# sc15i2gp/daily-ray-trace

Measured on AMD Instinct MI355X. Metric: Mpaths/s (pixels*spp/s) Cornell 1024^2 depth 8; achieved HBM GB/s % of peak, higher is better.
Workload: dtype f64

## Files before the change

daily-ray-trace_amd/csrc/drt_kernels.h:

```cpp
#pragma once

#include "drt_device.h"
#include "drt_build_rule.h"
#include "drt_stash_rule.h"
#include <type_traits>
#include "../../include/drt_hip.h"


enum
{
    SF_PX = 0, SF_PY, SF_PZ, SF_RADIUS,
    SF_NX, SF_NY, SF_NZ,
    SF_UNX, SF_UNY, SF_UNZ,
    SF_VNX, SF_VNY, SF_VNZ,
    SF_ULEN, SF_VLEN,
    SF_COUNT
};
enum
{
    LF_PX = 0, LF_PY, LF_PZ, LF_RADIUS,
    LF_UX, LF_UY, LF_UZ,
    LF_VX, LF_VY, LF_VZ,
    LF_PDF,
    LF_COUNT
// ... 1830 lines not shown
                                                     double ir, double tr, double te, double on_dot, double a_in, double spec,
                                                     double mn_dot, double ct_coef, uint32_t flags, bool paired)
{
    const uint64_t list = FIXED_N != 0u ? FIXED_LIST : list_arg;
    const uint32_t num_bdsfs = FIXED_N != 0u ? FIXED_N : num_bdsfs_arg;
    double bdsf_result = 0.0;
    double reflectance = 0.0;
#define DRT_PIN_HERE(x) asm volatile("" : "+v"(x))
    for (uint32_t i = 0; i < num_bdsfs; i += 1)
    {
        switch ((uint32_t)(list >> (4 * i)) & 15u)
        {
            case DRT_BDSF_bp_diffuse_bdsf:
                bdsf_result = diffuse_pi * a_in;
                break;
            case DRT_BDSF_bp_glossy_bdsf:
                bdsf_result = (glossy * spec) * a_in;
                break;
            case DRT_BDSF_mirror_bdsf:
                bdsf_result = (flags & FLAG_EQR) ? mirror : 0.0;
                break;
            case DRT_BDSF_fs_conductor_bdsf:
                if (SIMPLE) break;
                if (flags & FLAG_EQR)
                {
                    DRT_PIN_HERE(ir);
                    double c2 = on_dot * on_dot;
                    bdsf_result = conductor_reflectance_sel(paired, ir, tr, te, on_dot, c2, 1.0 - c2);
                }
                break;
            case DRT_BDSF_fs_dielectric_reflectance_bdsf:
                if (SIMPLE) break;
                if (flags & FLAG_EQR)
                {
                    DRT_PIN_HERE(ir);
                    bdsf_result = dielectric_reflectance_sel(paired, ir, tr, te, on_dot, 1.0 - on_dot * on_dot);
                }
                break;
            case DRT_BDSF_fs_dielectric_transmittance_bdsf:
                if (SIMPLE) break;
                if (flags & FLAG_EQT)
                {
                    DRT_PIN_HERE(ir);
                    bdsf_result = 1.0 - dielectric_reflectance_sel(paired, ir, tr, te, on_dot, 1.0 - on_dot * on_dot);
                }
                break;
            case DRT_BDSF_ct_conductor_bdsf:
            {
                if (SIMPLE) break;
                DRT_PIN_HERE(ir);
                double c2 = mn_dot * mn_dot;
                bdsf_result = conductor_reflectance_sel(paired, ir, tr, te, mn_dot, c2, 1.0 - c2) * ct_coef;
                break;
            }
            default: break;
        }
        reflectance = bdsf_result + reflectance;
    }
#undef DRT_PIN_HERE
    return reflectance;
}

#ifndef SHADE_PREFETCH_REGS
#define SHADE_PREFETCH_REGS 2
#endif
#define SHADE_PREFETCH_DEPTH 1
#define SHADE_PIXEL_CHUNK 16
#define TAIL_WINDOW_ENTRIES 112u
#define TAIL_WINDOW_WORDS (3u * TAIL_WINDOW_ENTRIES + TAIL_WINDOW_ENTRIES / 4u)
#define SHADE_WAVE_LDS_WORDS ((2u * 64u * SHADE_PREFETCH_REGS) > TAIL_WINDOW_WORDS ? (2u * 64u * SHADE_PREFETCH_REGS) : TAIL_WINDOW_WORDS)
#ifndef DRT_SHADE_CLOSED_LDS_HEADERS
#define DRT_SHADE_CLOSED_LDS_HEADERS 1
#endif
#define SHADE_CLOSED_SLOT_WORDS (64u * SHADE_PREFETCH_REGS)
#define SHADE_CLOSED_HDR01_AT SHADE_CLOSED_SLOT_WORDS
#define SHADE_CLOSED_HDR2_AT (SHADE_CLOSED_HDR01_AT + 128u)
#define SHADE_CLOSED_TAIL_ENTRIES 96u
#define SHADE_CLOSED_WAVE_LDS_WORDS (SHADE_CLOSED_HDR2_AT + 64u)
static_assert(3u * SHADE_CLOSED_TAIL_ENTRIES + SHADE_CLOSED_TAIL_ENTRIES / 4u <= SHADE_CLOSED_WAVE_LDS_WORDS, "the tail pass's window fits the closed form's region");
#define SHADE_WAVE_LDS_WORDS_FOR(closed_lds) ((closed_lds) ? SHADE_CLOSED_WAVE_LDS_WORDS : SHADE_WAVE_LDS_WORDS)

#define XYZ_FILM_WORDS 8

template <bool SPDS_IN_LDS, bool XYZ, bool SIMPLE, bool LIST = false>
__device__ __forceinline__ void shade_tail_group(const DevScene &sc, const ShadeParams &sp, const double *lds, uint64_t *wave_lds, const uint64_t *__restrict__ records,
                                                 const uint64_t *__restrict__ headers, double *__restrict__ film_pixels,
                                                 double *__restrict__ film_avgs, double *__restrict__ film_vars, uint64_t chunk_base,
                                                 uint64_t chunk_end, uint32_t lane, const bool closed, const bool closed_lds = false)
{
    const uint32_t S = sc.S;
    const uint32_t vw = sp.vertex_words;
    const uint32_t R = sp.tail_count;
    const uint32_t g = lane / R, j = lane - g * R;
    const bool act = g < (uint32_t)(chunk_end - chunk_base) && g < 64u / R;
    const uint32_t lam = sp.tail_first + j;
    const double *table = SPDS_IN_LDS ? (const double *)lds : sc.spds;
    const uint32_t n_groups = 64u / R;
    const uint32_t entries = closed_lds ? SHADE_CLOSED_TAIL_ENTRIES : TAIL_WINDOW_ENTRIES;
    const uint32_t win = entries / n_groups;
    uint16_t *task_list = (uint16_t *)(wave_lds + 3u * entries);
    const uint32_t leader = g * R;
    const bool in_group = g < n_groups;
    uint32_t v = 0, n_shaded = 0;
    uint64_t ph0 = 0;
    double vignette = 0.0, throughput = 1.0, dst = 0.0;
    uint64_t ph2 = 0;
    uint64_t slot = 0;
    const uint64_t *vcur = records;
    const bool one_light = sp.n_lights == 1u;
    const double em0 = spd_at(table, S, one_light ? sp.light0_em_spd : 0u, lam);
    auto deep_blocks = [&](uint32_t vertex) -> uint64_t { return vertex >= 2u * REC_BLOCK_VERTICES ? headers[slot * REC_HEADER_WORDS + 3] : 0ull; };
    for (uint32_t s0 = sp.tail_staged ? sp.n_samples : 0u; s0 < sp.n_samples; s0 += win)
    {
        const uint32_t s_end = s0 + win < sp.n_samples ? s0 + win : sp.n_samples;
        const uint32_t n_win = s_end - s0, n_px = (uint32_t)(chunk_end - chunk_base);
        uint32_t n_tasks = 0;
        for (uint32_t e0 = 0; e0 < n_px * n_win; e0 += 64u)
        {
            const uint32_t e = e0 + lane;
            const bool valid = e < n_px * n_win;
            const uint32_t ge = valid ? e / n_win : 0u, off = valid ? e - ge * n_win : 0u;
            const uint64_t eslot = (chunk_base + ge) * (uint64_t)sp.batch + s0 + off;
            uint64_t h0 = 0, h1 = 0, h2 = 0;
            if (valid)
            {
                const uint64_t *h = headers + eslot * REC_HEADER_WORDS;
                h0 = h[0];
                h1 = h[1];
                h2 = h[2];
            }
            const bool staged = ((uint32_t)(h0 >> 16) & HDR_TERM_TAIL_STAGED) != 0u;
            const bool has_path = valid && !staged && (h0 & 0xFFFFu) != 0u;
            if (valid && !staged && !has_path)
            {
                const bool emissive = ((uint32_t)(h0 >> 16) & HDR_TERM_MASK) == 1u;
                const uint32_t row = (uint32_t)(h0 >> 32) & 0xFFFFu;
                for (uint32_t t = 0; t < R; t += 1)
                {
                    double d = 0.0;
                    if (emissive) d = d + 1.0 * spd_at(table, S, row, sp.tail_first + t);
                    sp.tail_stage[eslot * R + t] = d * word_as_double(h1);
                }
            }
            const unsigned long long m = __ballot(has_path);
            if (has_path)
            {
                const uint32_t k = n_tasks + (uint32_t)__popcll(m & ((1ull << lane) - 1ull));
                task_list[k] = (uint16_t)e;
                uint64_t *w = wave_lds + e * 3u;
                w[0] = h0;
                w[1] = h1;
                w[2] = h2;
            }
            n_tasks += (uint32_t)__popcll(m);
        }
        __builtin_amdgcn_wave_barrier();
        uint32_t next_task = 0;
        bool busy = false;
        for (;;)
        {
            const unsigned long long want = __ballot(!busy && in_group && lane == leader);
            if (want != 0ull)
            {
                const uint32_t mine = next_task + (uint32_t)__popcll(want & ((1ull << leader) - 1ull));
                if (!busy && in_group && mine < n_tasks)
                {
                    const uint32_t e = task_list[mine];
                    const uint64_t *w = wave_lds + e * 3u;
                    const uint32_t ge = e / n_win, off = e - ge * n_win;
                    slot = (chunk_base + ge) * (uint64_t)sp.batch + s0 + off;
                    ph0 = w[0];
                    vignette = word_as_double(w[1]);
                    ph2 = w[2];
                    n_shaded = (uint32_t)(ph0 & 0xFFFFu);
                    const uint32_t k = ((uint32_t)(ph0 >> 16) >> HDR_TERM_RESUME_SHIFT) & HDR_TERM_RESUME_MASK;
                    v = k;
                    throughput = 1.0;
                    dst = 0.0;
                    if (k != 0u)
                    {
                        const double *at = sp.tail_stage + (slot * R + j);
                        dst = at[0];
                        throughput = at[shade_const().sp.tail_resume - sp.tail_stage];
                        vcur = path_vertex(records, sp.block_words, vw, ph2, deep_blocks(k), k);
                    }
                    else vcur = records + (uint64_t)(uint32_t)ph2 * sp.block_words;
                    busy = true;
                }
                next_task += (uint32_t)__popcll(want);
            }
            if (!__any(busy)) break;
            const bool has_vertex = busy && v < n_shaded;
            const bool is_plastic = has_vertex && v < 16u && (((uint32_t)(ph0 >> 48) >> v) & 1u);
            const bool is_general = has_vertex && !is_plastic;
            const uint32_t n_plastic = (uint32_t)__popcll(__ballot(is_plastic)), n_general = (uint32_t)__popcll(__ballot(is_general));
            if (n_plastic > 0 && n_plastic >= n_general)
            {
                if (is_plastic)
                {
                    const uint64_t *vrec = vcur;
                    const uint64_t w1 = vrec[1];
                    const double dir_pdf = word_as_double(vrec[4]);
                    const double s_a_in = word_as_double(vrec[5]), s_spec = word_as_double(vrec[6]);
                    const uint32_t i_diffuse = (uint32_t)(w1 >> 16) & 0xFFFFu, i_glossy = (uint32_t)(w1 >> 32) & 0xFFFFu;
                    const double diffuse_pi = spd_at(table, S, i_diffuse, lam), glossy = spd_at(table, S, i_glossy, lam);
                    double contribution = 0.0;
                    if (one_light && v < 8u)
                    {
                        if (((uint32_t)(ph0 >> 24) >> v) & 1u)
                        {
                            const uint64_t *lrec = vrec + REC_VERTEX_WORDS;
                            const double c = word_as_double(lrec[1]), a_in = word_as_double(lrec[2]), spec = word_as_double(lrec[3]);
                            double reflectance = diffuse_pi * a_in + 0.0;
                            reflectance = (glossy * spec) * a_in + reflectance;
                            contribution = contribution + reflectance;
                            contribution = contribution * em0;
                            contribution = contribution * c;
                        }
                    }
                    else if (one_light)
                    {
                        const uint64_t *lrec = vrec + REC_VERTEX_WORDS;
                        const uint64_t lw0 = lrec[0];
                        const double c = word_as_double(lrec[1]), a_in = word_as_double(lrec[2]), spec = word_as_double(lrec[3]);
                        double reflectance = diffuse_pi * a_in + 0.0;
                        reflectance = (glossy * spec) * a_in + reflectance;
                        double lit = 0.0 + reflectance;
                        lit = lit * em0;
                        lit = lit * c;
                        contribution = ((uint32_t)(lw0 >> 16) & FLAG_VISIBLE) ? lit : 0.0;
                    }
                    else
                    for (uint32_t l = 0; l < sp.n_lights; l += 1)
                    {
                        const uint64_t *lrec = vrec + REC_VERTEX_WORDS + l * REC_LIGHT_WORDS;
                        const uint64_t lw0 = lrec[0];
                        if (!((uint32_t)(lw0 >> 16) & FLAG_VISIBLE)) continue;
                        const double c = word_as_double(lrec[1]), a_in = word_as_double(lrec[2]), spec = word_as_double(lrec[3]);
                        double reflectance = diffuse_pi * a_in + 0.0;
                        reflectance = (glossy * spec) * a_in + reflectance;
                        contribution = contribution + reflectance;
                        contribution = contribution * spd_at(table, S, (uint32_t)(lw0 & 0xFFFFu), lam);
                        contribution = contribution * c;
                    }
                    dst = dst + throughput * contribution;
                    double reflectance = diffuse_pi * s_a_in + 0.0;
                    reflectance = (glossy * s_spec) * s_a_in + reflectance;
                    reflectance = reflectance * dir_pdf;
                    throughput = throughput * reflectance;
                    v += 1;
                    if (v < n_shaded) vcur = (v & (REC_BLOCK_VERTICES - 1u)) != 0u ? vcur + vw : path_vertex(records, sp.block_words, vw, ph2, deep_blocks(v), v);
                }
            }
            else if (n_general > 0)
            {
                if (is_general)
                {
                    const uint64_t *vrec = vcur;
                    const uint64_t list = vrec[0], w1 = vrec[1], w2 = vrec[2];
                    const double on_dot = word_as_double(vrec[3]), dir_pdf = word_as_double(vrec[4]);
                    const uint32_t num_bdsfs = (uint32_t)(w1 & 0xFFu);
                    const uint32_t sflags = (uint32_t)(w1 >> 8) & 0xFFu;
                    const uint32_t i_diffuse = (uint32_t)(w1 >> 16) & 0xFFFFu, i_glossy = (uint32_t)(w1 >> 32) & 0xFFFFu;
                    const double diffuse_pi = spd_at(table, S, i_diffuse, lam), glossy = spd_at(table, S, i_glossy, lam);
                    const double mirror = spd_at(table, S, (uint32_t)(w1 >> 48) & 0xFFFFu, lam);
                    uint32_t f0, f1, f2;
                    bool paired;
                    fresnel_rows(w2, f0, f1, f2, paired);
                    const double ir = SIMPLE ? 0.0 : spd_at(table, S, f0, lam), tr = SIMPLE ? 0.0 : spd_at(table, S, f1, lam), te = SIMPLE ? 0.0 : spd_at(table, S, f2, lam);
                    auto lane_vertex = [&](auto eval) {
                        double contribution = 0.0;
                        for (uint32_t l = 0; l < sp.n_lights; l += 1)
                        {
                            const uint64_t *lrec = vrec + REC_VERTEX_WORDS + l * REC_LIGHT_WORDS;
                            const uint64_t lw0 = lrec[0];
                            const uint32_t lflags = (uint32_t)(lw0 >> 16) & 0xFFu;
                            if (!(lflags & FLAG_VISIBLE)) continue;
                            double reflectance = eval(lflags, lrec + 2);
                            contribution = contribution + reflectance;
                            contribution = contribution * spd_at(table, S, (uint32_t)(lw0 & 0xFFFFu), lam);
                            contribution = contribution * word_as_double(lrec[1]);
                        }
                        dst = dst + throughput * contribution;
                        double reflectance = eval(sflags, vrec + 5);
                        reflectance = reflectance * dir_pdf;
                        throughput = throughput * reflectance;
                    };
                    const bool glass = !SIMPLE && num_bdsfs == 2u && list == DRT_LIST_GLASS;
                    const bool ggx = closed && list == DRT_LIST_GGX;
                    if (glass)
                        lane_vertex([&](uint32_t flags, const uint64_t *) {
                            return bdsf_at_wavelength<SIMPLE, 2, DRT_LIST_GLASS>(0, 0, 0.0, 0.0, 0.0, ir, tr, te, on_dot, 0.0, 0.0, 0.0, 0.0, flags, paired);
                        });
                    else if (ggx)
                        lane_vertex([&](uint32_t flags, const uint64_t *a) {
                            return bdsf_at_wavelength<SIMPLE, 1, DRT_LIST_GGX>(0, 0, 0.0, 0.0, 0.0, ir, tr, te, 0.0, 0.0, 0.0, word_as_double(a[2]), word_as_double(a[3]), flags, paired);
                        });
                    else if (closed && list == DRT_LIST_MIRROR)
                        lane_vertex([&](uint32_t flags, const uint64_t *) {
                            return bdsf_at_wavelength<SIMPLE, 1, DRT_LIST_MIRROR>(0, 0, 0.0, 0.0, mirror, 0.0, 0.0, 0.0, 0.0, 0.0, 0.0, 0.0, 0.0, flags, false);
                        });
                    else if (closed && list == DRT_LIST_CONDUCTOR)
                        lane_vertex([&](uint32_t flags, const uint64_t *) {
                            return bdsf_at_wavelength<SIMPLE, 1, DRT_LIST_CONDUCTOR>(0, 0, 0.0, 0.0, 0.0, ir, tr, te, on_dot, 0.0, 0.0, 0.0, 0.0, flags, paired);
                        });
                    else if (closed)
                        lane_vertex([&](uint32_t flags, const uint64_t *a) {
                            return bdsf_at_wavelength<SIMPLE, 2, DRT_LIST_PLASTIC>(0, 0, diffuse_pi, glossy, 0.0, 0.0, 0.0, 0.0, 0.0, word_as_double(a[0]), word_as_double(a[1]), 0.0, 0.0, flags, false);
                        });
                    else
                        lane_vertex([&](uint32_t flags, const uint64_t *a) {
                            return bdsf_at_wavelength<SIMPLE>(list, num_bdsfs, diffuse_pi, glossy, mirror, ir, tr, te, on_dot, word_as_double(a[0]), word_as_double(a[1]),
                                                              word_as_double(a[2]), word_as_double(a[3]), flags, paired);
                        });
                    v += 1;
                    if (v < n_shaded) vcur = (v & (REC_BLOCK_VERTICES - 1u)) != 0u ? vcur + vw : path_vertex(records, sp.block_words, vw, ph2, deep_blocks(v), v);
                }
            }
            if (busy && v >= n_shaded)
            {
                if (((uint32_t)(ph0 >> 16) & HDR_TERM_MASK) == 1u) dst = dst + throughput * spd_at(table, S, (uint32_t)(ph0 >> 32) & 0xFFFFu, lam);
                sp.tail_stage[slot * R + j] = dst * vignette;
                busy = false;
            }
        }
        __builtin_amdgcn_wave_barrier();
    }
    uint32_t j_b = j;
    asm volatile("" : "+v"(j_b));
    const uint32_t lam_b = sp.tail_first + j_b;
    uint32_t g_b = g;
    asm volatile("" : "+v"(g_b));
    const uint64_t pix_b = chunk_base + g_b;
    const uint64_t pix_f = LIST ? (act ? (uint64_t)sp.pixel_list[pix_b] : 0u) : pix_b;
    double *px = film_pixels + pix_f * (uint64_t)(XYZ ? XYZ_FILM_WORDS : S + 1);
    double *pa = XYZ ? nullptr : film_avgs + pix_f * (uint64_t)S;
    double *pv = XYZ ? nullptr : film_vars + pix_f * (uint64_t)S;
    const double *stage = sp.tail_stage + (pix_b * (uint64_t)sp.batch) * R + j_b;
    const uint32_t first = LIST ? sp.first_sample + (act ? sp.sample_base[pix_f] : 0u) : sp.first_sample;
    double f_sum = (act && !XYZ) ? px[lam_b] : 0.0, f_avg = (act && !XYZ) ? pa[lam_b] : 0.0, f_var = (act && !XYZ) ? pv[lam_b] : 0.0;
#pragma unroll 4
    for (uint32_t k = 0; k < sp.n_samples; k += 1)
    {
        const double contribution = act ? stage[(uint64_t)k * R] : 0.0;
        const double denom = (double)(first + k + 1);
        f_sum = f_sum + contribution;
        if (!XYZ)
        {
            double t0 = contribution - f_avg;
            double t1 = t0;
            t0 = t0 / denom;
            f_avg = f_avg + t0;
            t0 = contribution - f_avg;
            t0 = t1 * t0;
            f_var = f_var + t0;
        }
    }
    if (XYZ)
    {
        const double rw = spd_at(table, S, sp.cmf_rw, lam_b);
        const double x = act ? (spd_at(table, S, sp.cmf_x, lam_b) * f_sum * rw) : 0.0;
        const double y = act ? (spd_at(table, S, sp.cmf_y, lam_b) * f_sum * rw) : 0.0;
        const double z = act ? (spd_at(table, S, sp.cmf_z, lam_b) * f_sum * rw) : 0.0;
        double X = 0.0, Y = 0.0, Z = 0.0;
        for (uint32_t t = 0; t < R; t += 1)
        {
            const int src = (int)((lane - j_b + t) & 63u);
            X += __shfl(x, src);
            Y += __shfl(y, src);
            Z += __shfl(z, src);
        }
        if (act && j_b == 0)
        {
            px[4] += X;
            px[5] += Y;
            px[6] += Z;
        }
    }
    else if (act)
    {
        px[lam_b] = f_sum;
        pa[lam_b] = f_avg;
        pv[lam_b] = f_var;
    }
}


template <int NSETS, bool SPDS_IN_LDS, bool XYZ, bool DARK, bool SIMPLE, bool LIST, bool CLOSED, bool CLOSED_LDS = false>
__device__ __forceinline__ void shade_pixels(const DevScene &sc, const ShadeParams &sp, const uint64_t *__restrict__ records,
                                             const uint64_t *__restrict__ headers, double *__restrict__ film_pixels,
                                             double *__restrict__ film_avgs, double *__restrict__ film_vars,
                                             unsigned long long *__restrict__ work_counter)
{
    static_assert(!CLOSED || (NSETS == 1 && SPDS_IN_LDS && !XYZ && !SIMPLE && !LIST), "the closed form exists for one wavelength set, tables in LDS, spectral film, dense launches");
    extern __shared__ double lds[];
    const uint32_t S = sc.S;
    if (*sp.overflow) return;
    if (SPDS_IN_LDS)
    {
        const uint32_t spd_words = sc.n_spd * S;
        for (uint32_t k = threadIdx.x; k < spd_words; k += SHADE_BLOCK) lds[k] = sc.spds[k];
        __syncthreads();
    }
    const uint32_t lane_k = threadIdx.x & 63u;
    static_assert(!CLOSED_LDS || CLOSED, "the form with headers in LDS is a closed form");
    constexpr bool LDS_HDR = CLOSED_LDS;
    uint64_t *rec_lds = (uint64_t *)(lds + (SPDS_IN_LDS ? (size_t)sc.n_spd * S : 0)) + (size_t)(threadIdx.x >> 6) * SHADE_WAVE_LDS_WORDS_FOR(LDS_HDR);
    const uint32_t vw = sp.vertex_words;
    const uint32_t vpr = vw <= 64 ? 64u / vw : 0u;
    const uint32_t n_fast_regs = vpr * SHADE_PREFETCH_REGS;
    const uint32_t n_fast = n_fast_regs < 2u * REC_BLOCK_VERTICES ? n_fast_regs : 2u * REC_BLOCK_VERTICES;

    uint32_t lam_c[NSETS];
#pragma unroll
    for (int k = 0; k < NSETS; k += 1)
    {
        const uint32_t lam = 64u * k + lane_k;
        lam_c[k] = lam < S ? lam : 0;
    }

    const uint32_t S_main = sp.tail_count ? sp.tail_first : S;
    for (;;)
    {
        const ShadeParams &qc = shade_const().sp;
        uint32_t item = 0;
        if (lane_k == 0) item = (uint32_t)atomicAdd(work_counter, 1ull);
        item = (uint32_t)__builtin_amdgcn_readfirstlane((int)item);
        if (item >= qc.n_items) break;
        const uint32_t lane = made_again<LDS_HDR>(lane_k);
        if constexpr (LDS_HDR) lam_c[0] = lane < S ? lane : 0;
        const bool split = qc.items_per_group > 1;
        const bool inline_tail = qc.tail_count != 0;
        const uint32_t mains_per_group = qc.items_per_group - (inline_tail ? 1u : 0u);
        bool tail_item = inline_tail;
        uint32_t group = item, sub = 0;
        if (split)
        {
            uint32_t m = item;
            if (inline_tail)
            {
                const uint32_t n_groups = qc.n_items / qc.items_per_group;
                const uint32_t q = qc.tail_period_mains, mixed = n_groups * (q + 1u);
                if (item < mixed)
                {
                    const uint32_t period = item / (q + 1u), r = item - period * (q + 1u);
                    tail_item = r == 0u;
                    group = period;
                    m = period * q + (r - 1u);
                }
                else
                {
                    tail_item = false;
                    m = n_groups * q + (item - mixed);
                }
            }
            if (!tail_item)
            {
                group = m / mains_per_group;
                sub = m - group * mains_per_group;
            }
        }
        const uint64_t chunk_base = (uint64_t)group * qc.chunk;
        const uint64_t chunk_end = (chunk_base + qc.chunk < qc.n_pix) ? chunk_base + qc.chunk : qc.n_pix;
        uint64_t main_base = chunk_base, main_end = chunk_end;
        if (split)
        {
            main_base = chunk_base + (uint64_t)sub * qc.sub_pixels;
            main_end = (main_base + qc.sub_pixels < chunk_end) ? main_base + qc.sub_pixels : chunk_end;
            if (tail_item || main_base > chunk_end) main_base = main_end = chunk_end;
        }

      if (qc.mode == 2u) main_base = main_end;
      for (uint64_t pix = main_base; pix < main_end; pix += 1)
      {

        const uint64_t pix_f = LIST ? (uint64_t)sp.pixel_list[pix] : pix;
        double *px = film_pixels + pix_f * (uint64_t)(XYZ ? XYZ_FILM_WORDS : S + 1);
        double *pa = XYZ ? nullptr : film_avgs + pix_f * (uint64_t)S;
        double *pv = XYZ ? nullptr : film_vars + pix_f * (uint64_t)S;
        const uint32_t first = LIST ? sp.first_sample + sp.sample_base[pix_f] : sp.first_sample;
        double f_sum[NSETS], f_avg[NSETS], f_var[NSETS];
#pragma unroll
        for (int k = 0; k < NSETS; k += 1)
        {
            const uint32_t lam = 64u * k + lane;
            const bool active = lam < S_main;
            f_sum[k] = (active && !XYZ) ? px[lam] : 0.0;
            f_avg[k] = (active && !XYZ) ? pa[lam] : 0.0;
            f_var[k] = (active && !XYZ) ? pv[lam] : 0.0;
        }
        bool dark = false;
        if (DARK)
        {
            bool some = false;
#pragma unroll
            for (int k = 0; k < NSETS; k += 1)
                some = some || ((uint64_t)__double_as_longlong(f_sum[k]) | (uint64_t)__double_as_longlong(f_avg[k]) | (uint64_t)__double_as_longlong(f_var[k])) != 0ull;
            dark = !__any(some);
        }
      for (uint32_t s0 = 0; s0 < sp.n_samples; s0 += 64u)
      {
        const uint32_t n_win = (uint32_t)__builtin_amdgcn_readfirstlane((int)((sp.n_samples - s0 < 64u) ? sp.n_samples - s0 : 64u));
        __builtin_assume(n_win >= 1u);
        uint64_t h0 = 0, h1 = 0, h2 = 0, h3 = 0;
        if (lane < n_win)
        {
            const uint64_t *h = headers + (pix * sp.batch + s0 + lane) * REC_HEADER_WORDS;
            h0 = h[0];
            h1 = h[1];
            h2 = h[2];
            if (!LDS_HDR) h3 = h[3];
        }
        const unsigned long long worthless = !DARK ? 0ull : __ballot(lane < n_win && (h0 & 0xFFFFu) == 0ull && ((uint32_t)(h0 >> 16) & HDR_TERM_MASK) != 1u &&
                                                                      __builtin_isfinite(word_as_double(h1)));
        if (DARK && dark && (uint32_t)__popcll(worthless) == n_win) continue;
        auto prefetch_blocks = [&](uint64_t b2, uint32_t nw, uint64_t *dst) __attribute__((always_inline)) {
#pragma unroll
            for (int k = 0; k < SHADE_PREFETCH_REGS; k += 1)
            {
                const uint32_t b = (64u * k) >> (sp.vertex_shift + REC_BLOCK_SHIFT);
                const uint32_t id = b == 0 ? (uint32_t)b2 : (uint32_t)(b2 >> 32);
                const uint64_t *base = records + (uint64_t)id * sp.block_words + (64u * k - (b << (sp.vertex_shift + REC_BLOCK_SHIFT)));
                dst[k] = (64u * k + lane < nw) ? base[lane] : 0;
            }
        };
        auto prefetch = [&](uint32_t sa, uint32_t nw, uint64_t *dst) {
            if (nw == 0u) return;
            prefetch_blocks(readlane64(h2, sa), nw, dst);
        };
        uint64_t ring[SHADE_PREFETCH_DEPTH + 1][SHADE_PREFETCH_REGS];
        const uint64_t *hdr01 = rec_lds + SHADE_CLOSED_HDR01_AT, *hdr2 = rec_lds + SHADE_CLOSED_HDR2_AT;
        uint64_t hs_v = 0, vig_v = 0, nx0_v = 0, nx2_v = 0;
        auto fetch_headers = [&](uint32_t t) {
            const uint32_t a = t & 63u, b = (t + 1u) & 63u;
            hs_v = hdr01[a];
            vig_v = hdr01[64u + a];
            nx0_v = hdr01[b];
            nx2_v = hdr2[b];
        };
        if constexpr (LDS_HDR)
        {
            static_assert(SHADE_PREFETCH_DEPTH == 1, "one sample ahead");
            __builtin_amdgcn_wave_barrier();
            uint64_t *hw = rec_lds + SHADE_CLOSED_HDR01_AT;
            hw[lane] = h0;
            hw[64u + lane] = h1;
            hw[128u + lane] = h2;
            __builtin_amdgcn_wave_barrier();
            fetch_headers(0u);
            const uint64_t head0 = first64(hs_v);
            const uint32_t nw = (uint32_t)(head0 & 0xFFFFu) * vw;
            if (nw != 0u) prefetch_blocks(first64(hdr2[0]), nw, ring[1]);
        }
        else
        {
#pragma unroll
        for (int d = 0; d < SHADE_PREFETCH_DEPTH; d += 1)
        {
            const uint32_t nw = ((uint32_t)d < n_win) ? (uint32_t)(readlane64(h0, d) & 0xFFFFu) * vw : 0u;
            prefetch((uint32_t)d < n_win ? (uint32_t)d : 0u, nw, ring[d + 1]);
        }
        }
        for (uint32_t s = 0; s < n_win; s += 1)
        {
            const uint64_t hs = LDS_HDR ? first64(hs_v) : readlane64(h0, s);
            const uint64_t vig_w = LDS_HDR ? vig_v : readlane64(h1, s);
            const double vignette = word_as_double(vig_w);
            const uint32_t n_shaded = (uint32_t)(hs & 0xFFFFu);
            const uint32_t term = (uint32_t)(hs >> 16) & HDR_TERM_MASK;
// ... 399 lines not shown
                    for (int k = 0; k < NSETS; k += 1)
                    {
                        double reflectance = bdsf_at_wavelength<SIMPLE>(list, num_bdsfs, diffuse[k], glossy[k], mirror[k], ir[k], tr[k], te[k], on_dot,
                                                                word_as_double(lw[2]), word_as_double(lw[3]), word_as_double(lw[4]),
                                                                word_as_double(lw[5]), lflags, paired);
                        contribution[k] = contribution[k] + reflectance;
                        contribution[k] = contribution[k] * spd_at(table, S, i_em, lam_c[k]);
                        contribution[k] = contribution[k] * c;
                    }
                }
                const double s_mn = lifted_double<LDS_HDR>(vslot + 7, src, lane0 + 7), s_ct = lifted_double<LDS_HDR>(vslot + 8, src, lane0 + 8);
#pragma unroll
                for (int k = 0; k < NSETS; k += 1)
                {
                    dst[k] = dst[k] + throughput[k] * contribution[k];
                    double reflectance = bdsf_at_wavelength<SIMPLE>(list, num_bdsfs, diffuse[k], glossy[k], mirror[k], ir[k], tr[k], te[k], on_dot,
                                                            s_a_in, s_spec, s_mn, s_ct, sflags, paired);
                    reflectance = reflectance * dir_pdf;
                    throughput[k] = throughput[k] * reflectance;
                }
            }
            if constexpr (LDS_HDR) fetch_headers(s + 1u);
            const double denom = (double)(first + s0 + s + 1);
            if (DARK) dark = false;
#pragma unroll
            for (int k = 0; k < NSETS; k += 1)
            {
                if (term == 1)
                {
                    const double em = SPDS_IN_LDS ? spd_at((const double *)lds, S, term_spd, lam_c[k]) : spd_at(sc.spds, S, term_spd, lam_c[k]);
                    dst[k] = dst[k] + throughput[k] * em;
                }
                const double contribution = dst[k] * vignette;
                f_sum[k] = f_sum[k] + contribution;
                if (!XYZ)
                {
                    double t0 = contribution - f_avg[k];
                    double t1 = t0;
                    t0 = t0 / denom;
                    f_avg[k] = f_avg[k] + t0;
                    t0 = contribution - f_avg[k];
                    t0 = t1 * t0;
                    f_var[k] = f_var[k] + t0;
                }
            }
        }
      }
        if (XYZ)
        {
            const double *table = SPDS_IN_LDS ? (const double *)lds : sc.spds;
            double X = 0.0, Y = 0.0, Z = 0.0;
#pragma unroll
            for (int k = 0; k < NSETS; k += 1)
            {
                const uint32_t lam = 64u * k + lane;
                if (lam < S_main)
                {
                    const double rw = spd_at(table, S, sp.cmf_rw, lam);
                    X += (spd_at(table, S, sp.cmf_x, lam) * f_sum[k] * rw);
                    Y += (spd_at(table, S, sp.cmf_y, lam) * f_sum[k] * rw);
                    Z += (spd_at(table, S, sp.cmf_z, lam) * f_sum[k] * rw);
                }
            }
            for (int off = 32; off > 0; off >>= 1)
            {
                X += __shfl_xor(X, off);
                Y += __shfl_xor(Y, off);
                Z += __shfl_xor(Z, off);
            }
            if (lane == 0)
            {
                px[0] += X;
                px[1] += Y;
                px[2] += Z;
                px[3] += (double)sp.n_samples * 1.0;
            }
        }
        else
        {
#pragma unroll
            for (int k = 0; k < NSETS; k += 1)
            {
                const uint32_t lam = 64u * k + lane;
                if (lam < S_main)
                {
                    px[lam] = f_sum[k];
                    pa[lam] = f_avg[k];
                    pv[lam] = f_var[k];
                }
            }
            if (lane == 0) px[S] += (double)sp.n_samples * 1.0;
        }
      }

        if constexpr (LDS_HDR)
        {
            __builtin_amdgcn_wave_barrier();
        }
        if (tail_item && sp.mode != 1u) shade_tail_group<SPDS_IN_LDS, XYZ, SIMPLE, LIST>(sc, sp, (const double *)lds, rec_lds, records, headers, film_pixels, film_avgs, film_vars, chunk_base, chunk_end, made_again<LDS_HDR>(lane), CLOSED, LDS_HDR);
    }
}

template <int NSETS, bool SPDS_IN_LDS, bool XYZ, bool DARK, bool SIMPLE = false, bool LIST = false>
__global__ __launch_bounds__(SHADE_BLOCK, (SIMPLE && NSETS == 1) ? DRT_SHADE_WAVES_SIMPLE : SHADE_WAVES_PER_SIMD_FOR(NSETS)) void drt_shade_kernel(DevScene sc, ShadeParams sp, const uint64_t *__restrict__ records,
                                                                 const uint64_t *__restrict__ headers, double *__restrict__ film_pixels,
                                                                 double *__restrict__ film_avgs, double *__restrict__ film_vars,
                                                                 unsigned long long *__restrict__ work_counter)
{
    shade_pixels<NSETS, SPDS_IN_LDS, XYZ, DARK, SIMPLE, LIST, false>(sc, sp, records, headers, film_pixels, film_avgs, film_vars, work_counter);
}

#ifndef DRT_SHADE_WAVES_CLOSED
#define DRT_SHADE_WAVES_CLOSED 4
#endif
template <bool DARK>
__global__ __launch_bounds__(SHADE_BLOCK, DRT_SHADE_WAVES_CLOSED) void drt_shade_kernel_closed(DevScene sc, ShadeParams sp, const uint64_t *__restrict__ records,
                                                                 const uint64_t *__restrict__ headers, double *__restrict__ film_pixels,
                                                                 double *__restrict__ film_avgs, double *__restrict__ film_vars,
                                                                 unsigned long long *__restrict__ work_counter)
{
    shade_pixels<1, true, false, DARK, false, false, true>(sc, sp, records, headers, film_pixels, film_avgs, film_vars, work_counter);
}

#ifndef DRT_SHADE_WAVES_CLOSED_LDS
#define DRT_SHADE_WAVES_CLOSED_LDS 5
#endif
#if DRT_SHADE_CLOSED_LDS_HEADERS
template <bool DARK>
__global__ __launch_bounds__(SHADE_BLOCK, DRT_SHADE_WAVES_CLOSED_LDS) void drt_shade_kernel_closed_lds(DevScene sc, ShadeParams sp, const uint64_t *__restrict__ records,
                                                                 const uint64_t *__restrict__ headers, double *__restrict__ film_pixels,
                                                                 double *__restrict__ film_avgs, double *__restrict__ film_vars,
                                                                 unsigned long long *__restrict__ work_counter)
{
    shade_pixels<1, true, false, DARK, false, false, true, true>(sc, sp, records, headers, film_pixels, film_avgs, film_vars, work_counter);
}
#endif

__global__ void drt_film_xyz_kernel(DevScene sc, uint32_t cmf_rw, uint32_t cmf_x, uint32_t cmf_y, uint32_t cmf_z, double interval,
                                    uint64_t n_pix, const double *__restrict__ film_pixels, double *__restrict__ xyz)
{
    uint64_t p = (uint64_t)blockIdx.x * blockDim.x + threadIdx.x;
    if (p >= n_pix) return;
    const uint32_t S = sc.S;
    const double *rw = sc.spds + (size_t)cmf_rw * S, *cx = sc.spds + (size_t)cmf_x * S;
    const double *cy = sc.spds + (size_t)cmf_y * S, *cz = sc.spds + (size_t)cmf_z * S;
    const double *px = film_pixels + p * (uint64_t)(S + 1);
    double f = px[S];
    double n = 0.0;
    for (uint32_t i = 0; i < S; i += 1) n += (cy[i] * rw[i]);
    n *= interval;
    double X = 0.0, Y = 0.0, Z = 0.0;
    for (uint32_t i = 0; i < S; i += 1)
    {
        double v = px[i] / f;
        X += (cx[i] * v * rw[i]);
        Y += (cy[i] * v * rw[i]);
        Z += (cz[i] * v * rw[i]);
    }
    xyz[3 * p + 0] = X * (interval / n);
    xyz[3 * p + 1] = Y * (interval / n);
    xyz[3 * p + 2] = Z * (interval / n);
}

__global__ void drt_film_bgra_kernel(DevScene sc, uint32_t cmf_rw, uint32_t cmf_x, uint32_t cmf_y, uint32_t cmf_z, double interval,
                                     uint64_t n_pix, const double *__restrict__ film, int which, uint8_t *__restrict__ bgra)
{
    uint64_t p = (uint64_t)blockIdx.x * blockDim.x + threadIdx.x;
    if (p >= n_pix) return;
    const uint32_t S = sc.S;
    const double *rw = sc.spds + (size_t)cmf_rw * S, *cx = sc.spds + (size_t)cmf_x * S;
    const double *cy = sc.spds + (size_t)cmf_y * S, *cz = sc.spds + (size_t)cmf_z * S;
    const double *px = film + p * (uint64_t)(which == 0 ? S + 1 : S);
    double div = 1.0;
    bool divide = false;
    if (which == 0) { div = px[S]; divide = true; }
    if (which == 2)
    {
        double highest = 0.0;
        for (uint32_t i = 0; i < S; i += 1) if (px[i] > highest) highest = px[i];
        div = highest;
        divide = true;
    }
    double n = 0.0;
    for (uint32_t i = 0; i < S; i += 1) n += (cy[i] * rw[i]);
    n *= interval;
    double X = 0.0, Y = 0.0, Z = 0.0;
    for (uint32_t i = 0; i < S; i += 1)
    {
        double v = divide ? px[i] / div : px[i];
        X += (cx[i] * v * rw[i]);
        Y += (cy[i] * v * rw[i]);
        Z += (cz[i] * v * rw[i]);
    }
    X *= (interval / n);
    Y *= (interval / n);
    Z *= (interval / n);
    double rgb[3];
    rgb[0] = (2.3706743 * X) - (0.9000405 * Y) - (0.4706338 * Z);
    rgb[1] = (-0.5138850 * X) + (1.4253036 * Y) + (0.0885814 * Z);
    rgb[2] = (0.0052982 * X) - (0.0146949 * Y) + (1.0093968 * Z);
    uint8_t out[3];
    for (int c = 0; c < 3; c += 1)
    {
        double f = rgb[c];
        f = (f < 0.0) ? 0.0 : f;
        f = (f > 1.0) ? 1.0 : f;
        out[c] = (f == f) ? (uint8_t)(f * 255.0) : (uint8_t)0;
    }
    uchar4 o;
    o.x = out[2]; o.y = out[1]; o.z = out[0]; o.w = 255;
    ((uchar4 *)bgra)[p] = o;
}

__global__ void drt_xyz_finish_kernel(DevScene sc, uint32_t cmf_rw, uint32_t cmf_y, double interval, uint64_t n_pix,
                                      const double *__restrict__ film, double *__restrict__ xyz)
{
    uint64_t p = (uint64_t)blockIdx.x * blockDim.x + threadIdx.x;
// ... 313 lines not shown
```

daily-ray-trace_amd/csrc/drt_launcher.hip:

```cpp
#include "drt_kernels.h"
#include "drt_bvh_kernels.h"
#include "drt_adaptive_kernels.h"
#include "drt_sample_map_kernels.h"
#include "drt_denoise_kernels.h"
#include "drt_feature_kernels.h"
#include "drt_matte_kernels.h"
#include "drt_ray_kernels.h"
#include "drt_update_kernels.h"
#include "drt_build_kernels.h"
#include "drt_material_kernels.h"
#include "drt_depth_kernels.h"
#include "drt_sensor_kernels.h"
#include "drt_bucket_kernels.h"
#include "drt_lobe_kernels.h"
#include "drt_window_kernels.h"
#include "drt_window_rule.h"
#include "drt_pair_rule.h"
#include "drt_shade_lds_rule.h"
#include "drt_owned.h"

#include <algorithm>
#include <cmath>
#include <cstdarg>
#include <cstdio>
// ... 32 lines not shown

struct DeviceMem
{
    static std::atomic<uint64_t> &live() { static std::atomic<uint64_t> n{0}; return n; }
    static hipError_t alloc(void **p, size_t bytes)
    {
        const hipError_t e = hipMalloc(p, bytes);
        if (e == hipSuccess) live() += 1;
        return e;
    }
    static void free(void *p) { (void)hipFree(p); live() -= 1; }
};
struct PinnedMem
{
    static std::atomic<uint64_t> &live() { static std::atomic<uint64_t> n{0}; return n; }
    static hipError_t alloc(void **p, size_t bytes)
    {
        const hipError_t e = hipHostMalloc(p, bytes, hipHostMallocDefault);
        if (e == hipSuccess) live() += 1;
        return e;
    }
    static void free(void *p) { (void)hipHostFree(p); live() -= 1; }
};
template <typename T> using DevBuf = Owned<T, DeviceMem>;
template <typename T> using PinnedBuf = Owned<T, PinnedMem>;

struct drt_context
{
    int         device = 0;
    hipStream_t stream = nullptr;
    Stream      own_stream;
    drt_params  params{};
    DevScene    dsc{};
    DevCamera   dcam{};
    uint32_t    cmf_rw = 0, cmf_x = 0, cmf_y = 0, cmf_z = 0;
    double      interval = 0.0;

    std::vector<DevBuf<unsigned char>> allocations;
    std::vector<DevMaterial> host_mats;
    DevMaterial *d_mat_variants = nullptr;
    double *d_pixels = nullptr, *d_avgs = nullptr, *d_vars = nullptr;
    DevBuf<double> own_pixels, own_avgs, own_vars;
    bool    xyz_mode = false;
    bool    own_film = false;
    DevBuf<uint64_t> d_records, d_headers;
    uint32_t  light0_em_spd = 0;
    DevBuf<double> d_tail_stage;
    DevBuf<double> d_tail_resume;
    uint32_t  batch_spp = 1;
    uint32_t  vertex_words = 0, vertex_shift = 0, block_words = 0;
    uint64_t  pool_blocks = 0;
    uint32_t  worst_blocks_per_path = 0;
    double    est_blocks_per_path = 0.0;
    struct Batch { PairSpan span; uint64_t seq; };
    std::vector<Batch> inflight;
    uint64_t  next_seq = 1;
    uint64_t  redone_batches = 0, pool_peak = 0;
    DevBuf<int32_t> d_hits;
    uint64_t  hits_capacity = 0;
    uint32_t  hits_samples = 0;
    DevBuf<unsigned long long> d_counters;
    DevBuf<PrimaryHit> d_primary;
    DevBuf<uint64_t> d_queue;
    bool        bvh_pipeline = false;
    int         primary_grid_cap = 0, bounce_grid_cap = 0;
    DevBuf<double> d_xyz;
    DevBuf<uint8_t> d_bgra;
    bool      trace_tail = false;
    bool      tail_all_staged = false;
    bool      tail_resume = false;
    bool      dark_skip = true;
    bool      dark_skip_win = true;
    bool      no_fixed_lists = false;
    bool      simple_bdsfs = false;
    bool      no_closed_shade = false;
    bool      closed_lists = false;
    const double *d_spd_tail = nullptr;

    bool   scene_in_lds = true, spds_in_lds = true, use_bvh = false;
    size_t trace_lds = 0, shade_lds = 0;
    size_t shade_lds_closed = 0;
    bool   closed_lds = false;
    bool trace_stash = false;
    int    trace_grid_cap = 0, shade_grid_cap = 0;
    uint32_t trace_chunk_override = 0;
    ShadeOverrides shade_overrides;
    uint32_t debug_shade_mode = 0;
    bool     debug_tail_phase_a_off = false;
    uint32_t shade_sets = 1, tail_first = 0, tail_count = 0;
    uint64_t n_pix = 0;

    std::vector<Event> ev;
    std::vector<double> ev_paths;
    size_t ev_used = 0;
    double trace_ms = 0.0, shade_ms = 0.0;
    uint64_t timed_pairs = 0;
    double min_sample_ms = 0.0, max_sample_ms = 0.0, avg_sample_ms = 0.0;

    bool film_used = false, adaptive_done = false;
    DevBuf<uint32_t> d_counts;
    DevBuf<uint32_t> d_alist[2];
    DevBuf<unsigned long long> d_keep;
    DevBuf<uint32_t> d_bkeep;
    DevBuf<uint32_t> d_ainfo;
    PinnedBuf<uint32_t> h_active;
    uint64_t film_gen = 0;
    uint64_t dn_gen = 0;
    bool     dn_valid = false;
    DevBuf<double> d_dn_mean, d_dn_var, d_dn_guide, d_dn_weights, d_dn_wsum;
    DevBuf<uint32_t> d_dn_unusable;
    uint32_t dn_window_cap = 0;
    std::vector<drt_material> ft_mats;
    std::vector<double> ft_spds;
    uint32_t ft_n_spd = 0, ft_S = 0;
    DevBuf<double> d_ft_mean, d_ft_m2, d_ft_colour;
    DevBuf<int32_t> d_ft_ids;
    DevBuf<uint32_t> d_ft_counts, d_ft_report;
    DevBuf<unsigned long long> d_ft_info;
    Event    ft_ev[2];
    bool     ft_valid = false, ft_from_film = false;
    uint64_t ft_gen = 0;
    DevBuf<int32_t> d_mt_ids, d_mt_list;
    DevBuf<uint32_t> d_mt_counts, d_mt_tail;
    DevBuf<double> d_mt_cover;
    DevBuf<unsigned long long> d_mt_info;
    Event    mt_ev[2];
    bool     mt_valid = false, mt_from_film = false;
    uint64_t mt_gen = 0;
    uint64_t ray_chunk = RAY_STAGING_RAYS;
    int      ray_grid_cap = 1;
    DevBuf<double> d_ray_a, d_ray_b;
    DevBuf<drt_ray_hit> d_ray_hits;
    DevBuf<uint8_t> d_ray_visible;
    DevBuf<uint32_t> d_ray_xy, d_ray_samples;
    bool        rays_bound = false;
    DevRayTable rt{};
    DevBuf<double> d_rt_origins, d_rt_dirs, d_rt_weights;
    std::vector<drt_surface> h_surfaces;
    bool      h_stale = false;
    std::vector<BvhNode>  h_nodes;
    std::vector<uint32_t> h_order;
    double    cam_reach = 0.0, extent = 0.0;
    bool      extent_known = true;
    bool      upd_ready = false;
    DevBuf<drt_surface> d_raw; PinnedBuf<drt_surface> h_stage;
    DevBuf<int32_t> d_light_slot;
    DevBuf<double> d_boxes;
    DevBuf<uint32_t> d_leaf_parent;
    DevBuf<uint2> d_levels;
    std::vector<uint32_t> level_first;
    DevBuf<unsigned long long> d_upd_status;
    Event     upd_ev[3];
    bool      upd_timed = false, stage_busy = false;
    bool      upd_check = false, upd_violation = false;
    uint32_t  updates = 0, refits = 0;
    double    upd_ms = 0.0;
    bool      boxes_valid = false;
    bool      hb_ready = false, hb_timed = false;
    bool      hb_mirror_pending = false;
    DevBuf<uint32_t> d_hb_tree_surf, d_hb_pos[2], d_hb_table, d_hb_order;
    DevBuf<uint64_t> d_hb_keys[2];
    DevBuf<uint4> d_hb_items[2];
    DevBuf<unsigned char> d_hb_status; PinnedBuf<unsigned char> hb_mirror;
    Event     hb_ev[3];
    uint32_t  hb_builds = 0, hb_built_by = 0, hb_depth = 0;
    double    hb_ms = 0.0;
// ... 518 lines not shown
    if (ctx->use_bvh)
    {
        BvhBuilder bb;
        bb.build(scene, reach);
        if (bb.max_depth > BVH_STACK) return fail(-2, "BVH of %zu surfaces is %d levels deep, the traversal stack holds %d", bb.prims.size(), bb.max_depth, BVH_STACK);
        if (!(bb.extent < 134217728.0)) return fail(-2, "scene or camera coordinates reach %g: the hierarchy's f32 box test holds up to 2^27", bb.extent);
        std::vector<BvhLeafPrim> leaf(std::max<size_t>(bb.order.size(), 1));
        memset(leaf.data(), 0, leaf.size() * sizeof(BvhLeafPrim));
        for (size_t k = 0; k < bb.order.size(); k += 1)
        {
            const uint32_t i = bb.order[k];
            leaf[k].index = i;
            leaf[k].type = stype[i];
            for (int f = 0; f < 4; f += 1) leaf[k].f[f] = surf[(size_t)f * n_surf + i];
            leaf[k].reach32 = INFINITY;
            if (stype[i] == DRT_GEO_SPHERE)
            {
                for (int f = 0; f < 3; f += 1) leaf[k].c32[f] = (float)leaf[k].f[f];
                leaf[k].reach32 = bvh_sphere_reach32(leaf[k].f[3], bb.extent);
            }
        }
        if ((rc = upload(ctx, bb.nodes, &d.bvh_nodes))) return rc;
        if ((rc = upload(ctx, leaf, &d.bvh_leaf))) return rc;
        ctx->h_nodes = bb.nodes;
        ctx->h_order = bb.order;
        ctx->hb_depth = (uint32_t)bb.max_depth;
        ctx->extent = bb.extent;
    }
    if (!ctx->scene_in_lds) ctx->trace_lds = 0;
    ctx->spds_in_lds = (size_t)d.n_spd * S * 8 <= 64 * 1024;
    {
        uint32_t sets = 0, tf = 0, tc = 0;
        shade_sets(S, &sets, &tf, &tc);
        const size_t extra = (size_t)d.n_spd * tc * 8 + (size_t)(TRACE_BLOCK / 64) * (2 * tc + 1) * 64 * 8;
        ctx->simple_bdsfs = !getenv("DRT_NO_SIMPLE_SHADE");
        ctx->no_fixed_lists = getenv("DRT_NO_FIXED_LISTS") != nullptr;
        for (uint32_t i = 0; i < scene->num_materials; i += 1)
            for (uint32_t j = 0; j < mats[i].num_bdsfs; j += 1)
            {
                const uint32_t b = mats[i].bdsfs[j];
                if (b != DRT_BDSF_bp_diffuse_bdsf && b != DRT_BDSF_bp_glossy_bdsf && b != DRT_BDSF_mirror_bdsf) ctx->simple_bdsfs = false;
            }
        ctx->no_closed_shade = getenv("DRT_NO_CLOSED_SHADE") != nullptr;
        ctx->closed_lists = closed_lists(mats.data(), scene->num_materials, smat.data(), n_surf);
        bool all_simple = true;
        for (uint32_t i = 0; i < n_surf; i += 1)
        {
            const DevMaterial &m = mats[smat[i]];
            const bool mirror_only = m.num_bdsfs == 1u && m.bdsfs[0] == DRT_BDSF_mirror_bdsf;
            if (!(m.is_black_body || (m.vertex_flags & FLAG_PLASTIC) || mirror_only)) all_simple = false;
        }
        const char *e = getenv("DRT_TRACE_TAIL");
        const size_t lane_rows = (size_t)(TRACE_BLOCK / 64) * (TRACE_LANE_ROWS + 1) * 64 * 8;
        ctx->trace_tail = ctx->scene_in_lds && sets == 1 && tc > 0 && tc <= 8 && n_lights == 1 && ctx->trace_lds + extra - lane_rows <= 48 * 1024 && !(e && *e == '0') &&
                          (all_simple || !(e && *e == '2'));
        ctx->tail_all_staged = ctx->trace_tail && all_simple;
        const char *er = getenv("DRT_TAIL_RESUME");
        ctx->tail_resume = ctx->trace_tail && !ctx->tail_all_staged && !(er && *er == '0');
        if (ctx->trace_tail)
        {
            std::vector<double> cols((size_t)d.n_spd * tc);
            for (uint32_t r = 0; r < d.n_spd; r += 1)
                for (uint32_t j = 0; j < tc; j += 1) cols[(size_t)r * tc + j] = spds[(size_t)r * S + tf + j];
            if ((rc = upload(ctx, cols, &ctx->d_spd_tail))) return rc;
            ctx->trace_lds += extra;
        }
    }
    return 0;
}

static bool shade_simple(const drt_context *ctx) { return ctx->simple_bdsfs && ctx->spds_in_lds && ctx->shade_sets == 1; }

static bool shade_dark(const drt_context *ctx, const ShadeParams &sp)
{
    return (ctx->win_open && !sp.pixel_list) ? ctx->dark_skip_win : ctx->dark_skip;
}

static bool shade_closed(const drt_context *ctx)
{
    return ctx->closed_lists && !ctx->no_closed_shade && !ctx->no_fixed_lists && !shade_simple(ctx) && ctx->spds_in_lds && ctx->shade_sets == 1 && !ctx->xyz_mode;
}

static bool shade_closed_lds(const drt_context *ctx) { return DRT_SHADE_CLOSED_LDS_HEADERS != 0 && ctx->closed_lds && shade_closed(ctx); }

template <int NSETS, bool XYZ, bool LIST>
static int launch_shade_mode(drt_context *ctx, uint32_t grid, const ShadeParams &sp, double *const film[3])
{
    if (NSETS == 1 && !XYZ && !LIST && shade_closed(ctx))
    {
#define DRT_LAUNCH_CLOSED(KERNEL, DARK, LDS_BYTES)                                                                                                 \
    hipLaunchKernelGGL((KERNEL<DARK>), dim3(grid), dim3(SHADE_BLOCK), LDS_BYTES, ctx->stream, ctx->dsc, sp, ctx->d_records, \
                       ctx->d_headers, film[0], film[1], film[2], ctx->d_counters + DRT_NUM_COUNTERS + 1)
#if DRT_SHADE_CLOSED_LDS_HEADERS
        if (shade_closed_lds(ctx))
        {
            if (shade_dark(ctx, sp)) DRT_LAUNCH_CLOSED(drt_shade_kernel_closed_lds, true, ctx->shade_lds_closed);
            else DRT_LAUNCH_CLOSED(drt_shade_kernel_closed_lds, false, ctx->shade_lds_closed);
            return 0;
        }
#endif
        if (shade_dark(ctx, sp)) DRT_LAUNCH_CLOSED(drt_shade_kernel_closed, true, ctx->shade_lds);
        else DRT_LAUNCH_CLOSED(drt_shade_kernel_closed, false, ctx->shade_lds);
#undef DRT_LAUNCH_CLOSED
        return 0;
    }
#define DRT_LAUNCH_SHADE(LDS, DARK, SIMPLE)                                                                                                       \
    hipLaunchKernelGGL((drt_shade_kernel<NSETS, LDS, XYZ, DARK, SIMPLE, LIST>), dim3(grid), dim3(SHADE_BLOCK), ctx->shade_lds, ctx->stream, ctx->dsc, sp, \
                       ctx->d_records, ctx->d_headers, film[0], film[1], film[2], ctx->d_counters + DRT_NUM_COUNTERS + 1)
    if (NSETS == 1 && shade_simple(ctx))
    {
        if (shade_dark(ctx, sp)) DRT_LAUNCH_SHADE(true, true, (NSETS == 1));
        else DRT_LAUNCH_SHADE(true, false, (NSETS == 1));
    }
    else if (ctx->spds_in_lds && shade_dark(ctx, sp)) DRT_LAUNCH_SHADE(true, true, false);
    else if (ctx->spds_in_lds) DRT_LAUNCH_SHADE(true, false, false);
    else if (shade_dark(ctx, sp)) DRT_LAUNCH_SHADE(false, true, false);
    else DRT_LAUNCH_SHADE(false, false, false);
#undef DRT_LAUNCH_SHADE
    return 0;
}

template <int NSETS>
static int launch_shade_sets(drt_context *ctx, uint32_t grid, const ShadeParams &sp, double *const film[3])
{
    if (sp.pixel_list) return launch_shade_mode<NSETS, false, true>(ctx, grid, sp, film);
    return ctx->xyz_mode ? launch_shade_mode<NSETS, true, false>(ctx, grid, sp, film) : launch_shade_mode<NSETS, false, false>(ctx, grid, sp, film);
}

static void shade_sets(uint32_t S, uint32_t *n_sets, uint32_t *tail_first, uint32_t *tail_count)
{
    uint32_t full = S / 64, rem = S % 64;
    *tail_first = 0;
    *tail_count = 0;
    if (S <= 64 || rem == 0) *n_sets = (S + 63) / 64;
    else if (rem <= 16 && !getenv("DRT_NO_TAIL_PASS"))
    {
        *n_sets = full;
        *tail_first = 64 * full;
        *tail_count = rem;
    }
    else *n_sets = full + 1;
}

static int launch_shade(drt_context *ctx, uint32_t grid, const ShadeParams &sp, double *const film[3])
{
    switch (ctx->shade_sets)
    {
        case 1: return launch_shade_sets<1>(ctx, grid, sp, film);
        case 2: return launch_shade_sets<2>(ctx, grid, sp, film);
        case 3: return launch_shade_sets<3>(ctx, grid, sp, film);
        default: return launch_shade_sets<4>(ctx, grid, sp, film);
    }
}

template <int NCUTS>
static const void *depth_kernel(bool lds) { return lds ? (const void *)drt_depth_cut_kernel<NCUTS, true> : (const void *)drt_depth_cut_kernel<NCUTS, false>; }
static const void *depth_kernel(uint32_t n_cuts, bool lds)
{
    switch (n_cuts)
    {
        case 1: return depth_kernel<1>(lds);
        case 2: return depth_kernel<2>(lds);
        case 3: return depth_kernel<3>(lds);
        case 4: return depth_kernel<4>(lds);
        case 5: return depth_kernel<5>(lds);
        case 6: return depth_kernel<6>(lds);
        case 7: return depth_kernel<7>(lds);
        default: return depth_kernel<8>(lds);
    }
}
static size_t depth_lds_bytes(const drt_context *ctx) { return ctx->spds_in_lds ? (size_t)ctx->dsc.n_spd * ctx->dsc.S * 8 : 0; }

static int launch_depth_cuts(drt_context *ctx, const ShadeParams &sp, uint64_t pix0)
{
    const size_t S = ctx->dsc.S;
    DepthCutParams dp{};
// ... 321 lines not shown
    ctx->ft_spds.assign(scene->spds, scene->spds + (size_t)scene->num_spds * scene->num_wavelengths);
    if (const char *e = getenv("DRT_NO_LIVE_WINDOW")) ctx->win_allowed = atoi(e) == 0;
    if (ctx->xyz_mode)
    {
        const uint32_t rows[4] = {scene->cmf_rw, scene->cmf_x, scene->cmf_y, scene->cmf_z};
        for (int k = 0; k < 4; k += 1)
            for (uint32_t i = 0; i < scene->num_wavelengths; i += 1)
                if (!std::isfinite(scene->spds[(size_t)rows[k] * scene->num_wavelengths + i])) ctx->win_allowed = false;
    }

    set_device_camera(ctx, camera);

    const uint32_t S = scene->num_wavelengths;
    ctx->n_pix = (uint64_t)params->tile_w * params->tile_h;
    ctx->vertex_words = 16;
    while (ctx->vertex_words < REC_VERTEX_WORDS + REC_LIGHT_WORDS * ctx->dsc.n_lights) ctx->vertex_words *= 2;
    ctx->vertex_shift = 0;
    while ((1u << ctx->vertex_shift) < ctx->vertex_words) ctx->vertex_shift += 1;
    ctx->block_words = REC_BLOCK_VERTICES * ctx->vertex_words;
    const uint32_t deepest = (params->max_depth + REC_BLOCK_VERTICES - 1) / REC_BLOCK_VERTICES;
    ctx->worst_blocks_per_path = deepest + (deepest > REC_HEADER_BLOCKS ? 1u : 0u);
    if (deepest > REC_HEADER_BLOCKS + 2 * ctx->block_words)
        return fail(-2, "max_depth %u: a path's table block holds %u blocks beyond the header's %d", params->max_depth, 2 * ctx->block_words, REC_HEADER_BLOCKS);
    if (ctx->dsc.n_spd >= 0xFFFFu) return fail(-2, "too many SPDs for the 16-bit record indices");
    if (S > 64 * SHADE_MAX_SETS) return fail(-2, "more than %d wavelengths", 64 * SHADE_MAX_SETS);
    {
        uint32_t sets = 0, tf = 0, tc = 0;
        shade_sets(S, &sets, &tf, &tc);
        ctx->tail_count = tc;
    }
    ctx->bvh_pipeline = !ctx->scene_in_lds;

    HIP_TRY(ctx->own_pixels.need(pixels_bytes(ctx) / 8));
    if (!ctx->xyz_mode)
    {
        HIP_TRY(ctx->own_avgs.need((size_t)ctx->n_pix * S));
        HIP_TRY(ctx->own_vars.need((size_t)ctx->n_pix * S));
    }
    ctx->d_pixels = ctx->own_pixels;
    ctx->d_avgs = ctx->own_avgs;
    ctx->d_vars = ctx->own_vars;
    ctx->own_film = true;
    HIP_TRY(hipMemsetAsync(ctx->d_pixels, 0, pixels_bytes(ctx), ctx->stream));
    if (ctx->d_avgs) HIP_TRY(hipMemsetAsync(ctx->d_avgs, 0, (size_t)ctx->n_pix * S * 8, ctx->stream));
    if (ctx->d_vars) HIP_TRY(hipMemsetAsync(ctx->d_vars, 0, (size_t)ctx->n_pix * S * 8, ctx->stream));
    HIP_TRY(ctx->d_counters.need(DRT_COUNTER_WORDS));
    HIP_TRY(hipMemsetAsync(ctx->d_counters, 0, DRT_COUNTER_WORDS * sizeof(unsigned long long), ctx->stream));

    hipDeviceProp_t prop;
    HIP_TRY(hipGetDeviceProperties(&prop, ctx->device));
    int per_cu = 0;
    if (ctx->scene_in_lds && ctx->trace_tail)
        HIP_TRY(hipOccupancyMaxActiveBlocksPerMultiprocessor(&per_cu, drt_trace_direct_kernel<true, true>, TRACE_BLOCK, ctx->trace_lds));
    else if (ctx->scene_in_lds)
        HIP_TRY(hipOccupancyMaxActiveBlocksPerMultiprocessor(&per_cu, drt_trace_direct_kernel<true, false>, TRACE_BLOCK, ctx->trace_lds));
    ctx->trace_stash = false;
    if (ctx->scene_in_lds && !(getenv("DRT_NO_RAY_STASH") && atoi(getenv("DRT_NO_RAY_STASH")) != 0) && ctx->trace_lds + TRACE_STASH_BYTES <= 64 * 1024)
    {
        int with = 0;
        if (ctx->trace_tail) HIP_TRY(hipOccupancyMaxActiveBlocksPerMultiprocessor(&with, drt_trace_kernel<true, true>, TRACE_BLOCK, ctx->trace_lds + TRACE_STASH_BYTES));
        else HIP_TRY(hipOccupancyMaxActiveBlocksPerMultiprocessor(&with, drt_trace_kernel<true, false>, TRACE_BLOCK, ctx->trace_lds + TRACE_STASH_BYTES));
        ctx->trace_stash = with >= 1 && with >= per_cu;
    }
    if (per_cu < 1) per_cu = 1;
    if (const char *e = getenv("DRT_TRACE_BLOCKS_PER_CU")) per_cu = std::max(1, atoi(e));
    ctx->trace_grid_cap = prop.multiProcessorCount * per_cu;
    ctx->ray_grid_cap = prop.multiProcessorCount * 4;
    if (const char *e = getenv("DRT_RAY_CHUNK"))
        ctx->ray_chunk = std::max<uint64_t>(1, std::min<uint64_t>(RAY_STAGING_RAYS, strtoull(e, nullptr, 0)));
    if (ctx->bvh_pipeline)
    {
        int p_cu = 0, b_cu = 0;
        HIP_TRY(hipOccupancyMaxActiveBlocksPerMultiprocessor(&p_cu, drt_primary_kernel<false>, PRIMARY_BLOCK, 0));
        HIP_TRY(hipOccupancyMaxActiveBlocksPerMultiprocessor(&b_cu, drt_bounce_kernel<false>, BOUNCE_BLOCK, 0));
        if (const char *e = getenv("DRT_TRACE_BLOCKS_PER_CU")) b_cu = std::max(1, atoi(e));
        ctx->primary_grid_cap = prop.multiProcessorCount * std::max(1, p_cu);
        ctx->bounce_grid_cap = prop.multiProcessorCount * std::max(1, b_cu);
    }
    const ShadeLdsPlan lds_general = shade_lds_plan(ctx->dsc.n_spd, S, ctx->spds_in_lds, SHADE_WAVES, SHADE_WAVE_LDS_WORDS_FOR(false), DRT_SHADE_WAVES_PER_SIMD);
    const ShadeLdsPlan lds_closed = shade_lds_plan(ctx->dsc.n_spd, S, ctx->spds_in_lds, SHADE_WAVES, SHADE_WAVE_LDS_WORDS_FOR(true), DRT_SHADE_WAVES_CLOSED_LDS);
    ctx->shade_lds = lds_general.group_bytes;
    ctx->shade_lds_closed = lds_closed.group_bytes;
    ctx->closed_lds = lds_closed.groups >= DRT_SHADE_WAVES_CLOSED_LDS * SHADE_SIMDS_PER_CU / SHADE_WAVES && getenv("DRT_NO_CLOSED_LDS") == nullptr;
    int s_per_cu = 0;
    shade_sets(S, &ctx->shade_sets, &ctx->tail_first, &ctx->tail_count);
    switch (ctx->shade_sets)
    {
        case 1: rc = shade_occupancy<1>(ctx, &s_per_cu); break;
        case 2: rc = shade_occupancy<2>(ctx, &s_per_cu); break;
        case 3: rc = shade_occupancy<3>(ctx, &s_per_cu); break;
        default: rc = shade_occupancy<4>(ctx, &s_per_cu); break;
    }
    if (rc) return rc;
    const int s_query = s_per_cu;
    if (shade_closed_lds(ctx)) s_per_cu = std::min(s_per_cu, (int)lds_closed.groups);
    if (s_per_cu < 1) s_per_cu = 1;
    if (const char *e = getenv("DRT_SHADE_BLOCKS_PER_CU")) s_per_cu = std::max(1, atoi(e));
    ctx->shade_grid_cap = prop.multiProcessorCount * s_per_cu;
    if (const char *e = getenv("DRT_RESERVE_BLOCKS"))
    {
        int n = std::max(0, atoi(e));
        ctx->trace_grid_cap = std::max(1, ctx->trace_grid_cap - n);
        ctx->shade_grid_cap = std::max(1, ctx->shade_grid_cap - n);
    }
    if (const char *e = getenv("DRT_TRACE_CHUNK")) ctx->trace_chunk_override = (uint32_t)std::min(1 << 20, std::max(64, atoi(e) / 64 * 64));
    if (const char *e = getenv("DRT_TAIL_PERIOD")) ctx->shade_overrides.tail_period = (uint32_t)std::max(0, atoi(e));
    if (const char *e = getenv("DRT_SHADE_SUBS")) ctx->shade_overrides.subs = (uint32_t)std::max(0, atoi(e));
    if (const char *e = getenv("DRT_SHADE_CHUNK")) ctx->shade_overrides.chunk = (uint32_t)atoi(e);
    if (const char *e = getenv("DRT_DEBUG_SHADE_MODE")) ctx->debug_shade_mode = (uint32_t)atoi(e);
    if (const char *e = getenv("DRT_DEBUG_TAIL_PHASE_A_OFF")) ctx->debug_tail_phase_a_off = atoi(e) != 0;
    const size_t block_bytes = (size_t)ctx->block_words * 8;
    const uint64_t npx = std::max<uint64_t>(ctx->n_pix, 1);
    const size_t per_path_fixed = REC_HEADER_WORDS * 8 + (size_t)ctx->tail_count * 8 * (ctx->tail_resume ? 2 : 1) +
                                  (ctx->bvh_pipeline ? sizeof(PrimaryHit) + sizeof(uint64_t) : 0);
    size_t free_b = 0, total_b = 0;
    HIP_TRY(hipMemGetInfo(&free_b, &total_b));
    ctx->est_blocks_per_path = (double)ctx->worst_blocks_per_path;
    if (npx * (uint64_t)ctx->worst_blocks_per_path * block_bytes > (256ull << 20) && !getenv("DRT_POOL_WORST_CASE"))
    {
        const bool win = window_in_use(ctx);
        const PairWindow pw = {win, ctx->wx0, ctx->wx1, ctx->wy0, ctx->wy1};
        const uint64_t live_px = win ? (uint64_t)(ctx->wx1 - ctx->wx0) * (ctx->wy1 - ctx->wy0) : npx;
        const TraceTile sample = pool_sample_tile(ctx->params, pw, pool_sample_step(live_px));
        const uint64_t n_sample = sample.n_pix;
        ctx->pool_blocks = blocks_worst_case(ctx, n_sample);
        HIP_TRY(ctx->d_records.need(ctx->pool_blocks * ctx->block_words));
        HIP_TRY(ctx->d_headers.need(n_sample * REC_HEADER_WORDS));
        if (ctx->bvh_pipeline)
        {
            HIP_TRY(ctx->d_primary.need(n_sample));
            HIP_TRY(ctx->d_queue.need(n_sample));
        }
        if ((rc = enqueue_trace(ctx, sample, PairSpan::whole_tile(ctx->params.first_sample, 1, 0)))) return rc;
        unsigned long long used = 0;
        HIP_TRY(hipMemcpyAsync(&used, ctx->d_counters + DRT_PAIR_COUNTERS + 5, sizeof(used), hipMemcpyDeviceToHost, ctx->stream));
        HIP_TRY(hipStreamSynchronize(ctx->stream));
        ctx->est_blocks_per_path = (double)used / (double)n_sample * ((double)live_px / (double)npx);
        {
            unsigned long long cnt[3] = {0, 0, 0};
            HIP_TRY(hipMemcpy(cnt, ctx->d_counters + DRT_PAIR_COUNTERS, sizeof(cnt), hipMemcpyDeviceToHost));
            if (cnt[0] > 0)
            {
                const double per_path = (double)cnt[2] / (double)cnt[0];
                ctx->dark_skip_win = per_path < 3.0;
                ctx->dark_skip = per_path * ((double)live_px / (double)npx) < 3.0;
            }
        }
        ctx->d_records.reset();
        ctx->d_headers.reset();
        ctx->d_primary.reset();
        ctx->d_queue.reset();
        HIP_TRY(hipMemsetAsync(ctx->d_counters, 0, DRT_COUNTER_WORDS * sizeof(unsigned long long), ctx->stream));
        ctx->ev_used = 0;
        ctx->ev_paths.clear();
    }
    auto blocks_for = [&](uint64_t n_paths) -> uint64_t {
        const double want = 1.2 * ctx->est_blocks_per_path * (double)n_paths + 16.0 * std::sqrt((double)n_paths) + 4096.0;
        const uint64_t expect = (uint64_t)(want * (1.0 + 64.0 / POOL_CHUNK)) + trace_waves(ctx, n_paths) * (POOL_CHUNK + 2 * 64) + 1;
        return std::max<uint64_t>(std::min<uint64_t>(expect, blocks_worst_case(ctx, n_paths)), blocks_worst_case(ctx, npx));
    };
    uint32_t batch = params->batch_spp;
    if (batch == DRT_BATCH_RESIDENT)
    {
        const uint64_t resident_paths = getenv("DRT_RESIDENT_PATHS_M") ? (uint64_t)std::max(1, atoi(getenv("DRT_RESIDENT_PATHS_M"))) << 20 : (256ull << 20);
        const uint64_t by_paths = std::max<uint64_t>(1, std::min<uint64_t>(DRT_DEFAULT_MAX_BATCH, resident_paths / npx));
        batch = (uint32_t)std::max<uint64_t>(by_paths, 16);
        if (params->spp) batch = std::min(batch, params->spp);
    }
    else if (batch == 0)
    {
        const double path_bytes = 1.2 * (1.0 + 64.0 / POOL_CHUNK) * ctx->est_blocks_per_path * (double)block_bytes + (double)per_path_fixed;
        uint64_t by_job = (std::max<uint32_t>(params->spp, 1) + 31) / 32;
        uint64_t by_floor = (uint64_t)((double)(16ull << 30) / (path_bytes * (double)npx));
        uint64_t cap = std::max<uint64_t>(1, std::min<uint64_t>(DRT_DEFAULT_MAX_BATCH, (64ull << 20) / npx));
        batch = (uint32_t)std::max<uint64_t>(1, std::min(std::max(by_job, by_floor), cap));
        if (params->spp) batch = std::min(batch, params->spp);
    }
    batch = std::min<uint32_t>(batch, 4096);
    const size_t film_bytes = ctx->xyz_mode ? (size_t)ctx->n_pix * XYZ_FILM_WORDS * 8 : (size_t)ctx->n_pix * (3 * (size_t)S + 1) * 8;
    (void)film_bytes;
    auto bytes_for = [&](uint32_t b) -> size_t { return blocks_for(npx * b) * block_bytes + (size_t)npx * b * per_path_fixed; };
    while (batch > 1 && bytes_for(batch) > free_b / 2) batch /= 2;
    if (bytes_for(batch) > free_b) return fail(-3, "not enough device memory: need %zu bytes", bytes_for(batch));
    ctx->batch_spp = batch;
    ctx->pool_blocks = blocks_for(npx * batch);
    if (const char *e = getenv("DRT_POOL_BLOCKS"))
    {
        const bool win = window_in_use(ctx);
        const uint64_t live = (uint64_t)(ctx->wx1 - ctx->wx0) * (ctx->wy1 - ctx->wy0);
        const uint64_t floor_px = win ? std::min<uint64_t>(npx, std::max<uint64_t>(live, params->tile_w)) : npx;
        ctx->pool_blocks = std::max<uint64_t>(blocks_worst_case(ctx, floor_px), std::min<uint64_t>(ctx->pool_blocks, strtoull(e, nullptr, 0)));
    }
    if (ctx->pool_blocks >= 0xFFFFFFF0ull) return fail(-3, "record pool of %llu blocks: block numbers are 32 bits", (unsigned long long)ctx->pool_blocks);
    HIP_TRY(ctx->d_records.need(ctx->pool_blocks * ctx->block_words));
    HIP_TRY(ctx->d_headers.need((size_t)npx * batch * REC_HEADER_WORDS));
    if (ctx->bvh_pipeline)
    {
        HIP_TRY(ctx->d_primary.need((size_t)npx * batch));
        HIP_TRY(ctx->d_queue.need((size_t)npx * batch));
    }
    if (ctx->tail_count) HIP_TRY(ctx->d_tail_stage.need((size_t)npx * batch * ctx->tail_count));
    if (ctx->tail_count && ctx->tail_resume) HIP_TRY(ctx->d_tail_resume.need((size_t)npx * batch * ctx->tail_count));
    if (const char *e = getenv("DRT_DARK_SKIP")) ctx->dark_skip = ctx->dark_skip_win = atoi(e) != 0;
    if (getenv("DRT_VERBOSE"))
        fprintf(stderr, "drt: %d CUs, trace %d blocks/CU (lds %zu), shade %d blocks/CU (%s, occupancy query %d, lds %zu; LDS rule: general %u, closed %u of %zu bytes), batch %u, %.3f blocks/path measured (worst %u), pool %.2f GB\n",
                prop.multiProcessorCount, per_cu, ctx->trace_lds, s_per_cu, shade_closed_lds(ctx) ? "closed, headers in LDS" : shade_closed(ctx) ? "closed" : "general", s_query,
                shade_closed_lds(ctx) ? ctx->shade_lds_closed : ctx->shade_lds, lds_general.groups_by_lds, lds_closed.groups_by_lds, lds_closed.group_bytes,
                ctx->batch_spp, ctx->est_blocks_per_path,
                ctx->worst_blocks_per_path, (double)(ctx->pool_blocks * block_bytes) / 1e9);
    HIP_TRY(hipStreamSynchronize(ctx->stream));
    return 0;
}

extern "C" drt_context *drt_create(const drt_scene *scene, const drt_camera *camera, const drt_params *params)
{
    g_last_error.clear();
    drt_context *ctx = new drt_context();
    int rc = create_impl(ctx, scene, camera, params);
    if (rc != 0)
    {
        std::string keep = g_last_error;
        drt_destroy(ctx);
        (void)hipGetLastError();
        g_last_error = keep;
        return nullptr;
    }
    return ctx;
}

extern "C" void drt_destroy(drt_context *ctx)
{
    if (!ctx) return;
    (void)hipSetDevice(ctx->device);
    if (ctx->stream) (void)hipStreamSynchronize(ctx->stream);
    delete ctx;
}

extern "C" int drt_bind_film(drt_context *ctx, void *d_pixels, void *d_avgs, void *d_vars)
{
    if (!ctx || !d_pixels || (!ctx->xyz_mode && (!d_avgs || !d_vars))) return fail(-1, "null argument");
    HIP_TRY(hipSetDevice(ctx->device));
    HIP_TRY(hipStreamSynchronize(ctx->stream));
    ctx->own_pixels.reset();
    ctx->own_avgs.reset();
    ctx->own_vars.reset();
    ctx->own_film = false;
    ctx->film_gen += 1;
    ctx->d_pixels = (double *)d_pixels;
    ctx->d_avgs = (double *)d_avgs;
    ctx->d_vars = (double *)d_vars;
    return 0;
}

extern "C" int drt_set_stream(drt_context *ctx, void *hip_stream)
{
    if (!ctx) return fail(-1, "null context");
    HIP_TRY(hipSetDevice(ctx->device));
    HIP_TRY(hipStreamSynchronize(ctx->stream));
    ctx->stream = hip_stream ? (hipStream_t)hip_stream : ctx->own_stream;
    return 0;
}

extern "C" int drt_synchronize(drt_context *ctx);

static int next_events(drt_context *ctx, hipEvent_t out[3])
{
    if (ctx->ev.size() < ctx->ev_used + 3) ctx->ev.resize(ctx->ev_used + 3);
    for (int k = 0; k < 3; k += 1) HIP_TRY(ctx->ev[ctx->ev_used + k].need());
    for (int k = 0; k < 3; k += 1) out[k] = ctx->ev[ctx->ev_used + k];
    ctx->ev_used += 3;
    return 0;
}

static int collect_timings(drt_context *ctx)
{
    for (size_t k = 0; k + 3 <= ctx->ev_used; k += 3)
    {
        float a = 0.f, b = 0.f;
        HIP_TRY(hipEventElapsedTime(&a, ctx->ev[k], ctx->ev[k + 1]));
        HIP_TRY(hipEventElapsedTime(&b, ctx->ev[k + 1], ctx->ev[k + 2]));
        ctx->trace_ms += a;
        ctx->shade_ms += b;
        const double paths = k / 3 < ctx->ev_paths.size() ? ctx->ev_paths[k / 3] : 0.0;
        if (paths > 0.0)
        {
            const double t = ((double)a + (double)b) * (double)ctx->n_pix / paths;
// ... 133 lines not shown
    tp.spd_tail = ctx->d_spd_tail;
    tp.tail_count = ctx->tail_count;
    tp.n_spd = ctx->dsc.n_spd;
    unsigned long long *work = ctx->d_counters + DRT_NUM_COUNTERS;
    tp.pool_cursor = work + 4;
    tp.overflow = (uint32_t *)(work + 5);
    HIP_TRY(hipMemsetAsync(work, 0, 5 * sizeof(unsigned long long), ctx->stream));
    const uint32_t grid = trace_grid(tp.n_paths, TRACE_BLOCK, (uint32_t)(ctx->bvh_pipeline ? ctx->bounce_grid_cap : ctx->trace_grid_cap));
    tp.chunk = trace_chunk(tp.n_paths, grid, TRACE_BLOCK, ctx->bvh_pipeline, ctx->trace_chunk_override);
    DevRayTable rt = ctx->rt;
    rt.t_offset = tile.t_offset;
    const bool rays = ctx->rays_bound;
    if (ctx->bvh_pipeline)
    {
        const uint64_t packets = (tp.n_paths + 63) / 64;
        const uint32_t pgrid = (uint32_t)std::min<uint64_t>((packets + PRIMARY_BLOCK / 64 - 1) / (PRIMARY_BLOCK / 64), (uint64_t)ctx->primary_grid_cap);
#define DRT_BVH_ARGS_P ctx->dsc, ctx->dcam, tp, ctx->d_headers, ctx->d_hits, ctx->d_counters + DRT_PAIR_COUNTERS, ctx->d_primary, ctx->d_queue, work + 2
#define DRT_BVH_ARGS_B ctx->dsc, ctx->dcam, tp, ctx->d_records, ctx->d_headers, ctx->d_hits, ctx->d_counters + DRT_PAIR_COUNTERS, work, ctx->d_primary, ctx->d_queue, work + 2
#define DRT_LAUNCH_BVH(LIST)                                                                                                              \
        if (rays) hipLaunchKernelGGL(drt_primary_rays_kernel<LIST>, dim3(pgrid), dim3(PRIMARY_BLOCK), 0, ctx->stream, DRT_BVH_ARGS_P, rt); \
        else hipLaunchKernelGGL(drt_primary_kernel<LIST>, dim3(pgrid), dim3(PRIMARY_BLOCK), 0, ctx->stream, DRT_BVH_ARGS_P);               \
        HIP_TRY(hipGetLastError());                                                                                                       \
        if (rays) hipLaunchKernelGGL(drt_bounce_rays_kernel<LIST>, dim3(grid), dim3(BOUNCE_BLOCK), 0, ctx->stream, DRT_BVH_ARGS_B, rt);    \
        else hipLaunchKernelGGL(drt_bounce_kernel<LIST>, dim3(grid), dim3(BOUNCE_BLOCK), 0, ctx->stream, DRT_BVH_ARGS_B)
        if (list) { DRT_LAUNCH_BVH(true); }
        else { DRT_LAUNCH_BVH(false); }
#undef DRT_LAUNCH_BVH
#undef DRT_BVH_ARGS_P
#undef DRT_BVH_ARGS_B
    }
    else
    {
#define DRT_TRACE_ARGS ctx->dsc, ctx->dcam, tp, ctx->d_records, ctx->d_headers, ctx->d_hits, ctx->d_counters + DRT_PAIR_COUNTERS, work
#define DRT_LAUNCH_TRACE(TAIL, LIST)                                                                                                                       \
        if (rays) hipLaunchKernelGGL((drt_trace_rays_kernel<true, TAIL, LIST>), dim3(grid), dim3(TRACE_BLOCK), ctx->trace_lds, ctx->stream, DRT_TRACE_ARGS, rt); \
        else if (ctx->trace_stash) hipLaunchKernelGGL((drt_trace_kernel<true, TAIL, LIST>), dim3(grid), dim3(TRACE_BLOCK), ctx->trace_lds + TRACE_STASH_BYTES, ctx->stream, DRT_TRACE_ARGS); \
        else hipLaunchKernelGGL((drt_trace_direct_kernel<true, TAIL, LIST>), dim3(grid), dim3(TRACE_BLOCK), ctx->trace_lds, ctx->stream, DRT_TRACE_ARGS)
        const bool tail = ctx->trace_tail && tp.tail_stage;
        if (list && tail) { DRT_LAUNCH_TRACE(true, true); }
        else if (list) { DRT_LAUNCH_TRACE(false, true); }
        else if (tail) { DRT_LAUNCH_TRACE(true, false); }
        else { DRT_LAUNCH_TRACE(false, false); }
#undef DRT_LAUNCH_TRACE
#undef DRT_TRACE_ARGS
    }
    HIP_TRY(hipGetLastError());
    return 0;
}

static int enqueue_pair(drt_context *ctx, const PairSpan &span)
{
    hipEvent_t ev[3];
    int rc = next_events(ctx, ev);
    if (rc) return rc;
    ctx->film_gen += 1;
    HIP_TRY(hipEventRecord(ev[0], ctx->stream));
    const PairGeometry g = pair_geometry(span, ctx->params.tile_w, ctx->params.tile_h, pair_window(ctx));
    if (!g.windowed && (rc = pool_floor(ctx))) return rc;
    if (!g.nothing && (rc = enqueue_trace(ctx, pair_trace_tile(ctx->params, ctx->n_pix, ctx->batch_spp, span, g), span))) return rc;
    HIP_TRY(hipEventRecord(ev[1], ctx->stream));

    unsigned long long *work = ctx->d_counters + DRT_NUM_COUNTERS;
    ShadeParams sp{};
    sp.n_pix = g.n_pix;
    sp.n_samples = span.n_samples;
    sp.first_sample = span.first_sample;
    sp.vertex_words = ctx->vertex_words;
    sp.vertex_shift = ctx->vertex_shift;
    sp.block_words = ctx->block_words;
    sp.overflow = (const uint32_t *)(work + 5);
    sp.n_lights = ctx->dsc.n_lights;
    sp.batch = span.stride ? span.stride : ctx->batch_spp;
    sp.tail_first = ctx->tail_first;
    sp.tail_count = ctx->tail_count;
    sp.tail_stage = ctx->d_tail_stage;
    sp.tail_resume = ctx->d_tail_resume;
    sp.light0_em_spd = ctx->light0_em_spd;
    sp.no_fixed_lists = ctx->no_fixed_lists ? 1u : 0u;
    sp.tail_staged = ((ctx->tail_all_staged && ctx->d_tail_stage) || ctx->debug_tail_phase_a_off) ? 1u : 0u;
    sp.pixel_list = span.list;
    sp.sample_base = span.list ? ctx->d_counts : nullptr;
    sp.mode = ctx->debug_shade_mode;
    sp.cmf_rw = ctx->cmf_rw; sp.cmf_x = ctx->cmf_x; sp.cmf_y = ctx->cmf_y; sp.cmf_z = ctx->cmf_z;
    const ShadeQueue q = shade_queue(g.n_pix, span.n_samples, ctx->tail_count, sp.tail_staged, (uint32_t)ctx->shade_grid_cap, SHADE_WAVES, SHADE_PIXEL_CHUNK,
                                     ctx->shade_overrides);
    if (q.too_large) return fail(-1, "tile too large for the shade work queue");
    sp.chunk = q.chunk;
    sp.sub_pixels = q.sub_pixels;
    sp.items_per_group = q.items_per_group;
    sp.n_items = q.n_items;
    sp.tail_period_mains = q.tail_period_mains;
    const size_t S_ = ctx->dsc.S;
    const size_t film_words = ctx->xyz_mode ? (size_t)XYZ_FILM_WORDS : S_ + 1;
    double *const film[3] = {g.windowed ? ctx->d_win_film[0] + g.stage0 * film_words : ctx->d_pixels + g.pix0 * film_words,
                             g.windowed ? (ctx->xyz_mode ? nullptr : ctx->d_win_film[1] + g.stage0 * S_) : ctx->d_avgs ? ctx->d_avgs + g.pix0 * S_ : nullptr,
                             g.windowed ? (ctx->xyz_mode ? nullptr : ctx->d_win_film[2] + g.stage0 * S_) : ctx->d_vars ? ctx->d_vars + g.pix0 * S_ : nullptr};
    if (!g.nothing)
    {
        rc = launch_shade(ctx, q.grid, sp, film);
        if (rc) return rc;
        HIP_TRY(hipGetLastError());
    }
    if (ctx->n_cuts && (rc = launch_depth_cuts(ctx, sp, g.pix0))) return rc;
    if (ctx->n_sensor && (rc = launch_sensor(ctx, sp, g.pix0))) return rc;
    if (ctx->n_buckets && (rc = launch_buckets(ctx, sp, g.pix0))) return rc;
    if (ctx->n_lobes && (rc = launch_lobes(ctx, sp, g.pix0))) return rc;
    if (g.windowed && (rc = enqueue_window_fill(ctx, span.first_sample, span.n_samples, g.t_row0, g.t_rows))) return rc;
    const uint64_t seq = ctx->next_seq++;
    hipLaunchKernelGGL(drt_mark_pair_kernel, dim3(1), dim3(1), 0, ctx->stream, ctx->d_counters, (unsigned long long)seq);
    HIP_TRY(hipGetLastError());
    HIP_TRY(hipEventRecord(ev[2], ctx->stream));
    ctx->ev_paths.resize(ctx->ev_used / 3, 0.0);
    ctx->ev_paths[ctx->ev_used / 3 - 1] = (double)g.counted_paths;
    ctx->inflight.push_back({span, seq});
    return 0;
}

static int redo_batches(drt_context *ctx, uint64_t last_good_seq)
{
    std::vector<drt_context::Batch> todo;
    for (const auto &b : ctx->inflight) if (b.seq > last_good_seq) todo.push_back(b);
    ctx->inflight.clear();
    unsigned long long *work = ctx->d_counters + DRT_NUM_COUNTERS;
    HIP_TRY(hipMemsetAsync(work + 5, 0, sizeof(unsigned long long), ctx->stream));
    uint32_t safe = 1;
    while (safe < ctx->batch_spp && blocks_worst_case(ctx, ctx->n_pix * (uint64_t)(safe + 1)) <= ctx->pool_blocks) safe += 1;
    bool lists = false;
    for (const auto &b : todo) lists = lists || b.span.list != nullptr;
    const bool was_open = ctx->win_open;
    int rc = 0;
    if (lists) window_close(ctx);
    else if (!was_open) rc = window_open(ctx);
    if (!rc) rc = window_copy(ctx, true);
    if (rc) { ctx->win_open = was_open; return rc; }
    for (const auto &b : todo)
    {
        ctx->redone_batches += 1;
        for (uint32_t done = 0; done < b.span.n_samples; done += safe)
        {
            rc = enqueue_pair(ctx, b.span.narrowed(done, std::min(safe, b.span.n_samples - done)));
            if (rc) break;
        }
        if (rc) break;
    }
    {
        const int rc_back = window_copy(ctx, false);
        if (!rc) rc = rc_back;
        ctx->win_open = was_open;
    }
    if (rc) return rc;
    HIP_TRY(hipStreamSynchronize(ctx->stream));
    unsigned long long st[4] = {0, 0, 0, 0};
    HIP_TRY(hipMemcpy(st, work + 4, sizeof(st), hipMemcpyDeviceToHost));
    if ((uint32_t)st[1] != 0u) return fail(-6, "record pool exhausted in a launch sized for the worst case (%llu blocks)", (unsigned long long)ctx->pool_blocks);
    ctx->inflight.clear();
    return 0;
}

static int enqueue_blocks(drt_context *ctx, uint32_t first_sample, uint32_t num_samples, uint32_t n_blocks, std::vector<Event> *done)
{
    const uint32_t H = ctx->params.tile_h, W = ctx->params.tile_w;
    const uint32_t per = row_block_rows(H, n_blocks);
    const EqualSplit split = equal_split(num_samples, row_block_fit(num_samples, ctx->n_pix, ctx->batch_spp, per, W));
    for (uint32_t r0 = 0; r0 < H; r0 += per)
    {
        const uint32_t rows = std::min(per, H - r0);
        int rc = window_copy(ctx, true, r0, rows);
// ... 238 lines not shown
    int rc = film_to_bgra(ctx, which);
    if (rc) return rc;
    HIP_TRY(hipMemcpy(bgra, ctx->d_bgra, (size_t)ctx->n_pix * 4, hipMemcpyDeviceToHost));
    return 0;
}

extern "C" int drt_read_hit_indices(drt_context *ctx, int32_t *dst, uint64_t capacity_paths)
{
    if (!ctx || !dst) return fail(-1, "null argument");
    if (!(ctx->params.flags & DRT_FLAG_RECORD_HITS) || !ctx->d_hits) return fail(-4, "hit recording is off (DRT_FLAG_RECORD_HITS)");
    int rc = drt_synchronize(ctx);
    if (rc) return rc;
    uint64_t n = std::min<uint64_t>(capacity_paths, ctx->n_pix * (uint64_t)ctx->hits_samples);
    HIP_TRY(hipMemcpy(dst, ctx->d_hits, n * ctx->params.max_depth * sizeof(int32_t), hipMemcpyDeviceToHost));
    return 0;
}

extern "C" int drt_get_stats(drt_context *ctx, drt_stats *out)
{
    if (!ctx || !out) return fail(-1, "null argument");
    int rc = drt_synchronize(ctx);
    if (rc) return rc;
    unsigned long long c[DRT_NUM_COUNTERS];
    HIP_TRY(hipMemcpy(c, ctx->d_counters, sizeof(c), hipMemcpyDeviceToHost));
    memset(out, 0, sizeof(*out));
    out->paths = c[0];
    out->closest_hit_scans = c[1];
    out->shaded_vertices = c[2];
    out->shadow_scans = c[3];
    out->rng_draws = c[4];
    out->trace_ms = ctx->trace_ms;
    out->shade_ms = ctx->shade_ms;
    out->total_ms = ctx->trace_ms + ctx->shade_ms;
    out->record_pool_blocks = ctx->pool_blocks;
    out->record_pool_peak = ctx->pool_peak;
    out->record_block_bytes = ctx->block_words * 8;
    out->redone_launches = (uint32_t)ctx->redone_batches;
    out->launches = (uint32_t)std::min<uint64_t>(ctx->timed_pairs, 0xFFFFFFFFull);
    out->path_flags = (ctx->bvh_pipeline ? DRT_PATH_BVH : 0u) | ((ctx->trace_tail && ctx->d_tail_stage) ? DRT_PATH_TRACE_TAIL : 0u) |
                      (ctx->rays_bound ? DRT_PATH_RAYS : 0u) | ((ctx->trace_stash && !ctx->bvh_pipeline) ? DRT_PATH_RAY_STASH : 0u);
    out->min_sample_ms = ctx->min_sample_ms;
    out->max_sample_ms = ctx->max_sample_ms;
    out->avg_sample_ms = ctx->avg_sample_ms;
    return 0;
}

extern "C" uint32_t drt_batch_spp(drt_context *ctx) { return ctx ? ctx->batch_spp : 0; }

static void window_out(const LiveWindow &w, uint32_t out[4]) { out[0] = w.x_lo; out[1] = w.x_hi; out[2] = w.y_lo; out[3] = w.y_hi; }

extern "C" int drt_live_window_of(const drt_scene *scene, const drt_camera *camera, const drt_params *params, uint32_t out[4])
{
    g_last_error.clear();
    if (!scene || !camera || !params || !out) return fail(-1, "drt_live_window_of: null argument");
    if (scene->escape_material >= scene->num_materials) return fail(-2, "base/escape material index out of range");
    if ((uint64_t)params->x0 + params->tile_w > params->width ||
        (params->tile_h && (uint64_t)params->y0 + (uint64_t)(params->tile_h - 1) * (params->row_stride ? params->row_stride : 1) >= params->height))
        return fail(-1, "tile does not fit the %ux%u image", params->width, params->height);
    drt_params p = *params;
    if (p.row_stride == 0) p.row_stride = 1;
    window_out(live_window_of(scene->surfaces, scene->num_surfaces, scene->materials[scene->escape_material], *camera, p), out);
    return 0;
}

extern "C" int drt_live_window(drt_context *ctx, uint32_t out[4])
{
    if (!ctx || !out) return fail(-1, "drt_live_window: null argument");
    window_refresh(ctx);
    window_out(ctx->win, out);
    return 0;
}

extern "C" int drt_shade_instantiation(const drt_context *ctx)
{
    if (!ctx) return -1;
    if (shade_closed(ctx)) return DRT_SHADE_CLOSED;
    return shade_simple(ctx) ? DRT_SHADE_SIMPLE : DRT_SHADE_GENERAL;
}

extern "C" int drt_shade_closed_lds(const drt_context *ctx)
{
    if (!ctx) return -1;
    return shade_closed_lds(ctx) ? 1 : 0;
}

static int adaptive_check(drt_context *ctx, const drt_adaptive *a, bool held = false)
{
    if (!ctx || !a) return fail(-1, "null argument");
    if (ctx->n_cuts) return fail(-4, "adaptive sampling with depth cuts bound is not supported: drt_bind_depth_cuts(ctx, NULL, 0) first");
    if (ctx->n_sensor) return fail(-4, "adaptive sampling with a sensor bound is not supported: drt_bind_sensor(ctx, NULL, 0) first");
    if (ctx->n_buckets) return fail(-4, "adaptive sampling with buckets bound is not supported: drt_bind_buckets(ctx, 0) first");
    if (ctx->n_lobes) return fail(-4, "adaptive sampling with lobes bound is not supported: drt_bind_lobes(ctx, 0, NULL) first");
    if (ctx->xyz_mode) return fail(-4, "adaptive sampling needs the spectral film (DRT_MODE_XYZ keeps no variance)");
    if (ctx->params.flags & DRT_FLAG_RECORD_HITS) return fail(-4, "adaptive sampling does not record hit indices (DRT_FLAG_RECORD_HITS)");
    if (!held && ctx->adaptive_done) return fail(-7, "the film holds an adaptive render: drt_reset_film first");
    if (!held && ctx->film_used) return fail(-7, "adaptive sampling needs a film without samples: drt_reset_film first");
    if (held && !ctx->adaptive_done && !ctx->film_used) return fail(-7, "the film holds no samples to continue from: drt_render_adaptive renders from the start");
    if (a->min_spp < 2) return fail(-1, "min_spp %u: at least 2 (the variance needs two samples)", a->min_spp);
    if (a->max_spp < a->min_spp) return fail(-1, "max_spp %u is below min_spp %u", a->max_spp, a->min_spp);
    if (a->step < 1) return fail(-1, "step must be at least 1");
    if (a->flags != 0) return fail(-1, "flags %u: none are defined", a->flags);
    if (!std::isfinite(a->rel_error) || !(a->rel_error > 0.0)) return fail(-1, "rel_error %g: a finite number above 0", a->rel_error);
    if (!std::isfinite(a->floor) || !(a->floor >= 0.0)) return fail(-1, "floor %g: a finite number, 0 or more", a->floor);
    if (ctx->n_pix > 0xFFFFFFFFull) return fail(-1, "adaptive sampling lists pixels in 32 bits: the tile has %llu", (unsigned long long)ctx->n_pix);
    return 0;
}

static int enqueue_converge(drt_context *ctx)
{
    drt_context::Adaptive &ad = ctx->ad;
    const uint32_t n_blocks = (uint32_t)(((uint64_t)ad.n_in + CONVERGE_BLOCK - 1) / CONVERGE_BLOCK);
    ConvergeParams cp{};
    cp.list_in = ad.first ? nullptr : ctx->d_alist[ad.cur];
    cp.n_in = ad.n_in;
    cp.max_spp = ad.a.max_spp;
    cp.cmf_rw = ctx->cmf_rw;
    cp.cmf_y = ctx->cmf_y;
    cp.interval = ctx->interval;
    cp.rel_error = ad.a.rel_error;
    cp.floor = ad.a.floor;
    cp.counts = ctx->d_counts;
    cp.keep_mask = ctx->d_keep;
    cp.block_keep = ctx->d_bkeep;
    cp.active = ctx->d_bkeep + n_blocks;
    cp.list_out = ctx->d_alist[ad.cur ^ 1];
    cp.overflow = (const uint32_t *)(ctx->d_counters + DRT_NUM_COUNTERS + 5);
    cp.pixels = ctx->d_pixels;
    cp.at_max = ctx->d_ainfo;
    hipLaunchKernelGGL(drt_converge_kernel, dim3(n_blocks), dim3(CONVERGE_BLOCK), 0, ctx->stream, ctx->dsc, cp, ctx->d_avgs, ctx->d_vars);
    HIP_TRY(hipGetLastError());
    hipLaunchKernelGGL(drt_converge_scan, dim3(1), dim3(CONVERGE_SCAN_BLOCK), 0, ctx->stream, cp, n_blocks);
    HIP_TRY(hipGetLastError());
    hipLaunchKernelGGL(drt_converge_scatter, dim3(n_blocks), dim3(CONVERGE_BLOCK), 0, ctx->stream, cp);
    HIP_TRY(hipGetLastError());
    HIP_TRY(hipMemcpyAsync(ctx->h_active, cp.active, sizeof(uint32_t), hipMemcpyDeviceToHost, ctx->stream));
    HIP_TRY(hipMemcpyAsync(ctx->h_active + 1, ctx->d_ainfo, sizeof(uint32_t), hipMemcpyDeviceToHost, ctx->stream));
    return 0;
}

static int adaptive_alloc(drt_context *ctx)
{
    const uint64_t n_pix = ctx->n_pix;
    HIP_TRY(ctx->d_counts.need(n_pix));
    HIP_TRY(ctx->d_alist[0].need(n_pix));
    HIP_TRY(ctx->d_alist[1].need(n_pix));
    HIP_TRY(ctx->d_keep.need((n_pix + 63) / 64));
    HIP_TRY(ctx->d_bkeep.need((n_pix + CONVERGE_BLOCK - 1) / CONVERGE_BLOCK + 1));
    HIP_TRY(ctx->d_ainfo.need(1 + ADOPT_WORDS));
    HIP_TRY(ctx->h_active.need(2 + ADOPT_WORDS));
    return 0;
}

static int adaptive_buffers(drt_context *ctx)
{
    if (!ctx->h_active)
    {
        const int rc = adaptive_alloc(ctx);
        if (rc)
        {
            for (DevBuf<uint32_t> *b : {&ctx->d_counts, &ctx->d_alist[0], &ctx->d_alist[1], &ctx->d_bkeep, &ctx->d_ainfo}) b->reset();
            ctx->d_keep.reset();
            return rc;
        }
    }
    HIP_TRY(hipMemsetAsync(ctx->d_ainfo, 0, sizeof(uint32_t), ctx->stream));
    HIP_TRY(hipMemsetAsync(ctx->d_ainfo + 1 + ADOPT_BAD, 0xFF, sizeof(uint32_t), ctx->stream));
// ... 4042 lines not shown
```

daily-ray-trace_amd/csrc/drt_shade_lds_rule.h:

```cpp
#ifndef DRT_SHADE_LDS_RULE_H
#define DRT_SHADE_LDS_RULE_H

#include <algorithm>
#include <cstddef>
#include <cstdint>

#define SHADE_LDS_PER_CU (160u * 1024u)
#define SHADE_LDS_GRANULE 1280u
#define SHADE_SIMDS_PER_CU 4u

struct ShadeLdsPlan
{
    size_t   table_bytes;
    size_t   wave_bytes;
    size_t   group_bytes;
    size_t   granted_bytes;
    uint32_t groups_by_lds;
    uint32_t groups;
    uint32_t waves_per_simd;
};

static inline ShadeLdsPlan shade_lds_plan(uint32_t n_spd, uint32_t S, bool spds_in_lds, uint32_t block_waves, uint32_t wave_words, uint32_t register_waves)
{
    ShadeLdsPlan p{};
    p.table_bytes = spds_in_lds ? (size_t)n_spd * S * 8 : 0;
    p.wave_bytes = (size_t)wave_words * 8;
    p.group_bytes = p.table_bytes + (size_t)block_waves * p.wave_bytes;
    p.granted_bytes = (p.group_bytes + SHADE_LDS_GRANULE - 1) / SHADE_LDS_GRANULE * SHADE_LDS_GRANULE;
    p.groups_by_lds = p.granted_bytes ? (uint32_t)(SHADE_LDS_PER_CU / p.granted_bytes) : ~0u;
    const uint32_t groups_by_registers = register_waves * SHADE_SIMDS_PER_CU / std::max(1u, block_waves);
    p.groups = std::min(p.groups_by_lds, groups_by_registers);
    p.waves_per_simd = p.groups * block_waves / SHADE_SIMDS_PER_CU;
    return p;
}

#endif
```

daily-ray-trace_amd/pydrt.py:

```python
import ctypes as C
import os
import sys

import numpy as np

HERE = os.path.dirname(os.path.abspath(__file__))
REPO = os.path.dirname(HERE)

DRT_MAX_BDSFS = 16
GEO_POINT, GEO_SPHERE, GEO_PLANE = 1, 2, 3
FILM_SAMPLE_CENTER, FILM_SAMPLE_RANDOM = 1, 2
MODE_SPECTRAL, MODE_XYZ = 0, 1
FLAG_RECORD_HITS = 1
BATCH_RESIDENT = 0xFFFFFFFF
FLAG_FILM_ZERO = 2
PATH_BVH, PATH_TRACE_TAIL, PATH_RAYS, PATH_RAY_STASH = 1, 2, 4, 8

BDSF_NAMES = ["bp_diffuse_bdsf", "bp_glossy_bdsf", "mirror_bdsf", "fs_conductor_bdsf",
              "fs_dielectric_reflectance_bdsf", "fs_dielectric_transmittance_bdsf", "ct_conductor_bdsf"]
DIRF_NAMES = ["cos_weighted_sample_hemisphere", "uniform_sample_hemisphere", "sample_specular_direction",
              "sample_transmit_direction", "sample_reflect_or_transmit_direction", "sample_ct_direction"]
BDSF = {n: i for i, n in enumerate(BDSF_NAMES)}
DIRF = {n: i for i, n in enumerate(DIRF_NAMES)}

# ... 563 lines not shown
        if not os.path.exists(path):
            raise RuntimeError("libdrt_hip.so is not built (no fallback exists): run __graft_entry__.build()")
        _share_torch_hip_runtime()
        L = C.CDLL(path)
        L.drt_last_error.restype = C.c_char_p
        L.drt_device_count.restype = C.c_int
        L.drt_create.restype = C.c_void_p
        L.drt_create.argtypes = [C.POINTER(Scene), C.POINTER(Camera), C.POINTER(Params)]
        L.drt_destroy.argtypes = [C.c_void_p]
        L.drt_bind_film.argtypes = [C.c_void_p, C.c_void_p, C.c_void_p, C.c_void_p]
        L.drt_set_stream.argtypes = [C.c_void_p, C.c_void_p]
        L.drt_render.argtypes = [C.c_void_p, C.c_uint32, C.c_uint32]
        L.drt_synchronize.argtypes = [C.c_void_p]
        L.drt_reset_film.argtypes = [C.c_void_p]
        L.drt_film_device_ptrs.argtypes = [C.c_void_p, C.POINTER(C.c_void_p), C.POINTER(C.c_void_p), C.POINTER(C.c_void_p)]
        L.drt_read_film.argtypes = [C.c_void_p, C.POINTER(C.c_double), C.POINTER(C.c_double), C.POINTER(C.c_double)]
        L.drt_read_xyz.argtypes = [C.c_void_p, C.POINTER(C.c_double)]
        L.drt_read_bgra.argtypes = [C.c_void_p, C.c_int, C.POINTER(C.c_uint8)]
        L.drt_group_read_bgra.argtypes = [C.c_void_p, C.c_int, C.POINTER(C.c_uint8)]
        f64p, i32p = C.POINTER(C.c_double), C.POINTER(C.c_int32)
        L.drt_group_create.restype = C.c_void_p
        L.drt_group_create.argtypes = [C.POINTER(Scene), C.POINTER(Camera), C.POINTER(Params), i32p, C.c_uint32]
        L.drt_group_destroy.argtypes = [C.c_void_p]
        L.drt_group_destroy.restype = None
        L.drt_group_size.argtypes = [C.c_void_p]
        L.drt_group_size.restype = C.c_uint32
        L.drt_group_render.argtypes = [C.c_void_p, C.c_uint32, C.c_uint32]
        L.drt_group_synchronize.argtypes = [C.c_void_p]
        L.drt_group_read_film.argtypes = [C.c_void_p, f64p, f64p, f64p]
        L.drt_group_write_film.argtypes = [C.c_void_p, f64p, f64p, f64p]
        L.drt_group_get_stats.argtypes = [C.c_void_p, C.POINTER(Stats)]
        L.drt_render_tile_multi.argtypes = [C.POINTER(Scene), C.POINTER(Camera), C.POINTER(Params), i32p, C.c_uint32, f64p, f64p, f64p,
                                            C.POINTER(Stats)]
        L.drt_write_film.argtypes = [C.c_void_p, C.POINTER(C.c_double), C.POINTER(C.c_double), C.POINTER(C.c_double)]
        L.drt_read_hit_indices.argtypes = [C.c_void_p, C.POINTER(C.c_int32), C.c_uint64]
        L.drt_get_stats.argtypes = [C.c_void_p, C.POINTER(Stats)]
        L.drt_render_adaptive.argtypes = [C.c_void_p, C.POINTER(Adaptive)]
        L.drt_read_sample_counts.argtypes = [C.c_void_p, C.POINTER(C.c_uint32)]
        L.drt_read_active_list.argtypes = [C.c_void_p, C.POINTER(C.c_uint32), C.c_uint32, C.POINTER(C.c_uint32)]
        L.drt_group_render_adaptive.argtypes = [C.c_void_p, C.POINTER(Adaptive)]
        L.drt_group_read_sample_counts.argtypes = [C.c_void_p, C.POINTER(C.c_uint32)]
        L.drt_render_adaptive_continue.argtypes = [C.c_void_p, C.POINTER(Adaptive), C.c_uint32, C.POINTER(C.c_uint32)]
        L.drt_group_render_adaptive_continue.argtypes = [C.c_void_p, C.POINTER(Adaptive), C.c_uint32, C.POINTER(C.c_uint32)]
        if hasattr(L, "drt_render_sample_map"):
            L.drt_render_sample_map.argtypes = [C.c_void_p, C.POINTER(SampleMap)]
            L.drt_group_render_sample_map.argtypes = [C.c_void_p, C.POINTER(SampleMap)]
        if hasattr(L, "drt_denoise_film"):
            L.drt_denoise_film.argtypes = [C.c_void_p, C.POINTER(Denoise)]
            L.drt_read_denoised.argtypes = [C.c_void_p, f64p, f64p]
            L.drt_read_denoised_bgra.argtypes = [C.c_void_p, C.POINTER(C.c_uint8)]
            L.drt_denoise_buffers.argtypes = [C.POINTER(Scene), C.POINTER(Params), C.POINTER(Denoise), f64p, f64p, f64p, f64p, f64p]
            L.drt_group_denoise.argtypes = [C.c_void_p, C.POINTER(Denoise), f64p, f64p]
        if hasattr(L, "drt_render_features"):
            L.drt_render_features.argtypes = [C.c_void_p, C.POINTER(Features)]
            L.drt_read_features.argtypes = [C.c_void_p, f64p, f64p, i32p]
            L.drt_read_feature_bgra.argtypes = [C.c_void_p, C.c_int, C.c_double, C.c_double, C.POINTER(C.c_uint8)]
            L.drt_group_render_features.argtypes = [C.c_void_p, C.POINTER(Features), f64p, f64p, i32p]
        if hasattr(L, "drt_cast_rays"):
            vp = C.c_void_p
            L.drt_cast_rays.argtypes = [C.c_void_p, vp, vp, C.c_uint64, vp, C.c_uint32]
            L.drt_test_visibility.argtypes = [C.c_void_p, vp, vp, C.c_uint64, vp, C.c_uint32]
            L.drt_cast_pixels.argtypes = [C.c_void_p, vp, vp, C.c_uint64, vp, vp, vp, C.c_uint32]
            L.drt_group_cast_rays.argtypes = [C.c_void_p, vp, vp, C.c_uint64, vp]
            L.drt_group_test_visibility.argtypes = [C.c_void_p, vp, vp, C.c_uint64, vp]
            L.drt_group_cast_pixels.argtypes = [C.c_void_p, vp, vp, C.c_uint64, vp, vp, vp]
        if hasattr(L, "drt_render_mattes"):
            u32p = C.POINTER(C.c_uint32)
            L.drt_render_mattes.argtypes = [C.c_void_p, C.POINTER(Mattes)]
            L.drt_read_mattes.argtypes = [C.c_void_p, i32p, u32p, u32p]
            L.drt_read_matte.argtypes = [C.c_void_p, C.c_int, i32p, C.c_uint32, f64p]
            L.drt_read_matte_bgra.argtypes = [C.c_void_p, C.c_int, C.POINTER(C.c_uint8)]
            L.drt_group_render_mattes.argtypes = [C.c_void_p, C.POINTER(Mattes), i32p, u32p, u32p]
        L.drt_batch_spp.restype = C.c_uint32
        if hasattr(L, "drt_bind_rays"):
            L.drt_bind_rays.argtypes = [C.c_void_p, C.POINTER(RayTable)]
            L.drt_group_bind_rays.argtypes = [C.c_void_p, C.POINTER(RayTable)]
        L.drt_batch_spp.argtypes = [C.c_void_p]
        if hasattr(L, "drt_shade_instantiation"):
            L.drt_shade_instantiation.argtypes = [C.c_void_p]
            L.drt_shade_instantiation.restype = C.c_int
        if hasattr(L, "drt_shade_closed_lds"):
            L.drt_shade_closed_lds.argtypes = [C.c_void_p]
            L.drt_shade_closed_lds.restype = C.c_int
        if hasattr(L, "drt_update_surfaces"):
            L.drt_set_camera.argtypes = [C.c_void_p, C.POINTER(Camera)]
            L.drt_update_surfaces.argtypes = [C.c_void_p, C.c_void_p, C.c_uint32, C.c_uint32, C.c_uint32]
            L.drt_get_update_report.argtypes = [C.c_void_p, C.POINTER(UpdateReport)]
            L.drt_group_set_camera.argtypes = [C.c_void_p, C.POINTER(Camera)]
            L.drt_group_update_surfaces.argtypes = [C.c_void_p, C.c_void_p, C.c_uint32, C.c_uint32, C.c_uint32]
            L.drt_group_reset_film.argtypes = [C.c_void_p]
        if hasattr(L, "drt_update_spectra"):
            L.drt_update_spectra.argtypes = [C.c_void_p, C.c_void_p, C.c_uint32, C.c_uint32, C.c_uint32]
            L.drt_update_materials.argtypes = [C.c_void_p, C.c_void_p, C.c_uint32, C.c_uint32, C.c_uint32]
            L.drt_group_update_spectra.argtypes = [C.c_void_p, C.c_void_p, C.c_uint32, C.c_uint32, C.c_uint32]
            L.drt_group_update_materials.argtypes = [C.c_void_p, C.c_void_p, C.c_uint32, C.c_uint32, C.c_uint32]
        if hasattr(L, "drt_bind_depth_cuts"):
            u32p, vpp = C.POINTER(C.c_uint32), C.POINTER(C.c_void_p)
            L.drt_bind_depth_cuts.argtypes = [C.c_void_p, u32p, C.c_uint32]
            L.drt_read_depth_film.argtypes = [C.c_void_p, C.c_uint32, f64p, f64p, f64p]
            L.drt_depth_film_device_ptrs.argtypes = [C.c_void_p, C.c_uint32, vpp, vpp, vpp]
            L.drt_read_depth_xyz.argtypes = [C.c_void_p, C.c_uint32, f64p]
            L.drt_read_depth_bgra.argtypes = [C.c_void_p, C.c_uint32, C.c_int, C.POINTER(C.c_uint8)]
            L.drt_group_bind_depth_cuts.argtypes = [C.c_void_p, u32p, C.c_uint32]
            L.drt_group_read_depth_film.argtypes = [C.c_void_p, C.c_uint32, f64p, f64p, f64p]
        if hasattr(L, "drt_bind_sensor"):
            vpp = C.POINTER(C.c_void_p)
            L.drt_bind_sensor.argtypes = [C.c_void_p, f64p, C.c_uint32]
            L.drt_read_sensor_film.argtypes = [C.c_void_p, f64p, f64p, f64p]
            L.drt_sensor_film_device_ptrs.argtypes = [C.c_void_p, vpp, vpp, vpp]
            L.drt_read_sensor_bgra.argtypes = [C.c_void_p, C.c_int, f64p, C.POINTER(C.c_uint8)]
            L.drt_group_bind_sensor.argtypes = [C.c_void_p, f64p, C.c_uint32]
            L.drt_group_read_sensor_film.argtypes = [C.c_void_p, f64p, f64p, f64p]
        if hasattr(L, "drt_bind_buckets"):
            vpp, u8p = C.POINTER(C.c_void_p), C.POINTER(C.c_uint8)
            L.drt_bind_buckets.argtypes = [C.c_void_p, C.c_uint32]
            L.drt_read_bucket_film.argtypes = [C.c_void_p, C.c_uint32, f64p, f64p, f64p]
            L.drt_bucket_film_device_ptrs.argtypes = [C.c_void_p, C.c_uint32, vpp, vpp, vpp]
            L.drt_resolve_buckets.argtypes = [C.c_void_p, C.c_uint32]
            L.drt_read_bucket_resolve.argtypes = [C.c_void_p, f64p, f64p]
            L.drt_bucket_resolve_device_ptrs.argtypes = [C.c_void_p, vpp, vpp]
            L.drt_read_bucket_resolve_xyz.argtypes = [C.c_void_p, f64p]
            L.drt_read_bucket_resolve_bgra.argtypes = [C.c_void_p, u8p]
            L.drt_group_bind_buckets.argtypes = [C.c_void_p, C.c_uint32]
            L.drt_group_read_bucket_film.argtypes = [C.c_void_p, C.c_uint32, f64p, f64p, f64p]
            L.drt_group_resolve_buckets.argtypes = [C.c_void_p, C.c_uint32]
            L.drt_group_read_bucket_resolve.argtypes = [C.c_void_p, f64p, f64p]
        if hasattr(L, "drt_bind_lobes"):
            vpp, u8p, mapp = C.POINTER(C.c_void_p), C.POINTER(C.c_uint8), C.POINTER(LobeMap)
            L.drt_bind_lobes.argtypes = [C.c_void_p, C.c_uint32, mapp]
            L.drt_read_lobe_film.argtypes = [C.c_void_p, C.c_uint32, f64p, f64p, f64p]
            L.drt_lobe_film_device_ptrs.argtypes = [C.c_void_p, C.c_uint32, vpp, vpp, vpp]
            L.drt_read_lobe_xyz.argtypes = [C.c_void_p, C.c_uint32, f64p]
            L.drt_read_lobe_bgra.argtypes = [C.c_void_p, C.c_uint32, C.c_int, u8p]
            L.drt_group_bind_lobes.argtypes = [C.c_void_p, C.c_uint32, mapp]
            L.drt_group_read_lobe_film.argtypes = [C.c_void_p, C.c_uint32, f64p, f64p, f64p]
        if hasattr(L, "drt_rebuild_hierarchy"):
            L.drt_rebuild_hierarchy.argtypes = [C.c_void_p, C.c_uint32]
            L.drt_group_rebuild_hierarchy.argtypes = [C.c_void_p, C.c_uint32]
            L.drt_get_hierarchy_report.argtypes = [C.c_void_p, C.POINTER(HierarchyReport)]
            L.drt_read_hierarchy.argtypes = [C.c_void_p, C.c_void_p, C.c_uint32, C.POINTER(C.c_uint32), C.c_uint32]
        if hasattr(L, "drt_live_window_of"):
            L.drt_live_window_of.argtypes = [C.POINTER(Scene), C.POINTER(Camera), C.POINTER(Params), C.POINTER(C.c_uint32)]
            L.drt_live_window.argtypes = [C.c_void_p, C.POINTER(C.c_uint32)]
        L.drt_render_tile.argtypes = [C.POINTER(Scene), C.POINTER(Camera), C.POINTER(Params), C.POINTER(C.c_double),
                                      C.POINTER(C.c_double), C.POINTER(C.c_double), C.POINTER(Stats)]
        L.drt_selftest_arith.argtypes = [C.c_int, C.c_int, C.POINTER(C.c_double), C.POINTER(C.c_double),
                                         C.POINTER(C.c_double), C.c_uint64]
        if hasattr(L, "drt_selftest_path_ids"):
            L.drt_selftest_path_ids.argtypes = [C.c_int, C.POINTER(C.c_uint64), C.c_uint32, C.POINTER(C.c_uint32), C.c_uint32, C.c_uint32,
                                                C.c_uint32, C.POINTER(C.c_uint64)]
        L.drt_bvh_stats.argtypes = [C.POINTER(Scene)] + [C.POINTER(C.c_uint32)] * 4
        L.drt_selftest_unit.argtypes = [C.c_int, C.c_int, C.POINTER(C.c_double), C.c_uint32, C.POINTER(C.c_double), C.c_uint32,
                                        C.c_uint64]
        L.drt_selftest_material.argtypes = [C.c_void_p, C.c_int, C.POINTER(C.c_double), C.c_uint32, C.POINTER(C.c_double), C.c_uint32,
                                            C.c_uint64]
        if hasattr(L, "drt_selftest_build_sort"):
            u32p, u64p = C.POINTER(C.c_uint32), C.POINTER(C.c_uint64)
            L.drt_selftest_build_sort.argtypes = [C.c_int, u64p, C.c_uint32, u64p, u32p]
            L.drt_selftest_build_topology.argtypes = [C.c_int, u64p, C.c_uint32, C.POINTER(C.c_int32), C.POINTER(C.c_int32), u32p, u32p]
        if hasattr(L, "drt_selftest_live_resources"):
            L.drt_selftest_live_resources.argtypes = [C.POINTER(C.c_uint64)]
        if hasattr(L, "drt_selftest_division"):
            L.drt_selftest_division.argtypes = [C.c_int, C.c_int, C.POINTER(C.c_double), C.c_uint32, C.POINTER(C.c_double), C.c_uint32,
                                                C.c_uint64]
        _hip = L
    return _hip


SHADE_INSTANTIATIONS = ("general", "simple", "closed")

HIP_SYMBOLS = ["drt_shade_instantiation", "drt_shade_closed_lds",
               "drt_last_error", "drt_device_count", "drt_create", "drt_destroy", "drt_bind_film", "drt_set_stream",
               "drt_render", "drt_synchronize", "drt_reset_film", "drt_film_device_ptrs", "drt_read_film", "drt_write_film",
               "drt_read_xyz", "drt_read_bgra", "drt_read_hit_indices", "drt_get_stats", "drt_batch_spp", "drt_render_tile", "drt_selftest_arith",
               "drt_selftest_unit", "drt_selftest_material", "drt_selftest_path_ids", "drt_bvh_stats",
               "drt_selftest_build_sort", "drt_selftest_build_topology", "drt_selftest_live_resources",
               "drt_group_create", "drt_group_destroy", "drt_group_size", "drt_group_render", "drt_group_synchronize",
               "drt_group_read_film", "drt_group_write_film", "drt_group_read_bgra", "drt_group_get_stats", "drt_render_tile_multi",
               "drt_render_adaptive", "drt_read_sample_counts", "drt_group_render_adaptive", "drt_group_read_sample_counts",
               "drt_read_active_list", "drt_render_adaptive_continue", "drt_group_render_adaptive_continue",
               "drt_denoise_film", "drt_read_denoised", "drt_read_denoised_bgra", "drt_denoise_buffers", "drt_group_denoise",
               "drt_render_features", "drt_read_features", "drt_read_feature_bgra", "drt_group_render_features",
               "drt_render_mattes", "drt_read_mattes", "drt_read_matte", "drt_read_matte_bgra", "drt_group_render_mattes",
               "drt_cast_rays", "drt_test_visibility", "drt_cast_pixels", "drt_group_cast_rays", "drt_group_test_visibility",
               "drt_group_cast_pixels", "drt_bind_rays", "drt_group_bind_rays",
               "drt_set_camera", "drt_update_surfaces", "drt_get_update_report", "drt_group_set_camera", "drt_group_update_surfaces",
               "drt_group_reset_film",
               "drt_rebuild_hierarchy", "drt_group_rebuild_hierarchy", "drt_get_hierarchy_report", "drt_read_hierarchy",
               "drt_update_spectra", "drt_update_materials", "drt_group_update_spectra", "drt_group_update_materials",
               "drt_bind_depth_cuts", "drt_read_depth_film", "drt_depth_film_device_ptrs", "drt_read_depth_xyz", "drt_read_depth_bgra",
               "drt_group_bind_depth_cuts", "drt_group_read_depth_film",
               "drt_bind_sensor", "drt_read_sensor_film", "drt_sensor_film_device_ptrs", "drt_read_sensor_bgra",
               "drt_group_bind_sensor", "drt_group_read_sensor_film",
               "drt_bind_buckets", "drt_read_bucket_film", "drt_bucket_film_device_ptrs", "drt_resolve_buckets", "drt_read_bucket_resolve",
               "drt_bucket_resolve_device_ptrs", "drt_read_bucket_resolve_xyz", "drt_read_bucket_resolve_bgra",
               "drt_group_bind_buckets", "drt_group_read_bucket_film", "drt_group_resolve_buckets", "drt_group_read_bucket_resolve",
               "drt_bind_lobes", "drt_read_lobe_film", "drt_lobe_film_device_ptrs", "drt_read_lobe_xyz", "drt_read_lobe_bgra",
               "drt_group_bind_lobes", "drt_group_read_lobe_film",
               "drt_render_sample_map", "drt_group_render_sample_map",
               "drt_live_window_of", "drt_live_window", "drt_selftest_division"]

MAX_DEPTH_CUTS = 8


def _depth_array(depths):
    depths = [] if depths is None else [int(d) for d in depths]
    if any(d < 0 or d > 0xFFFFFFFF for d in depths):
        raise ValueError("bind_depth_cuts: depths are unsigned 32-bit numbers")
    return ((C.c_uint32 * len(depths))(*depths) if depths else None), len(depths)


MAX_SENSOR_CHANNELS = 8


def _sensor_curves(curves, S):
    if curves is None:
        return None, 0
    a = np.ascontiguousarray(curves, dtype=np.float64)
    if a.ndim == 1 and a.size == 0:
        return None, 0
    if a.ndim != 2 or a.shape[1] != S:
        raise ValueError("bind_sensor: curves of shape %s, need [n][%d] (one value per wavelength of the render's grid)" % (a.shape, S))
    if a.shape[0] == 0:
        return None, 0
    return a, int(a.shape[0])


def _sensor_matrix(matrix, n):
    m = np.ascontiguousarray(matrix, dtype=np.float64)
    if m.shape != (3, n):
        raise ValueError("read_sensor_bgra: a matrix of shape %s, need (3, %d): the bound channels to R, G, B" % (m.shape, n))
    return m


MAX_BUCKETS = 8


def _u32(value, what):
    v = int(value)
    if v < 0 or v > 0xFFFFFFFF:
        raise ValueError("%s = %d: an unsigned 32-bit number" % (what, v))
    return v


def bucket_pair(means):
    m = np.asarray(means, dtype=np.float64)
    if m.ndim < 1 or m.shape[0] < 2:
        raise ValueError("bucket_pair: means of shape %s, need [n][...] with n >= 2 buckets" % (m.shape,))
    out = []
    for half in (m[0::2], m[1::2]):
        acc = half[0].copy()
        for k in range(1, half.shape[0]):
            acc = acc + half[k]
        out.append(acc / float(half.shape[0]))
# ... 246 lines not shown

    def read_bucket_resolve_xyz(self):
        out = np.empty((self.n_pixels, 3))
        _check(self.L.drt_read_bucket_resolve_xyz(self.ctx, _ptr(out, C.c_double)), "drt_read_bucket_resolve_xyz")
        return out

    def read_bucket_resolve_bgra(self):
        out = np.empty((self.n_pixels, 4), dtype=np.uint8)
        _check(self.L.drt_read_bucket_resolve_bgra(self.ctx, _ptr(out, C.c_uint8)), "drt_read_bucket_resolve_bgra")
        return out

    def bind_lobes(self, map_or_preset, n=None):
        n, m = _lobe_bind_args(map_or_preset, n)
        _check(self.L.drt_bind_lobes(self.ctx, n, C.byref(m) if m is not None else None), "drt_bind_lobes")
        self.n_lobes = n

    def read_lobe_film(self, c):
        c = _u32(c, "read_lobe_film: c")
        if not getattr(self, "n_lobes", 0) or c >= self.n_lobes:
            _check(self.L.drt_read_lobe_film(self.ctx, c, None, None, None), "drt_read_lobe_film")
        S, n = self.S, self.n_pixels
        px, av, va = np.empty((n, S + 1)), np.empty((n, S)), np.empty((n, S))
        _check(self.L.drt_read_lobe_film(self.ctx, c, _ptr(px, C.c_double), _ptr(av, C.c_double), _ptr(va, C.c_double)), "drt_read_lobe_film")
        return px, av, va

    def lobe_film_device_ptrs(self, c):
        a, b, d = C.c_void_p(), C.c_void_p(), C.c_void_p()
        _check(self.L.drt_lobe_film_device_ptrs(self.ctx, _u32(c, "lobe_film_device_ptrs: c"), C.byref(a), C.byref(b), C.byref(d)),
               "drt_lobe_film_device_ptrs")
        return a.value, b.value, d.value

    def read_lobe_xyz(self, c):
        out = np.empty((self.n_pixels, 3))
        _check(self.L.drt_read_lobe_xyz(self.ctx, _u32(c, "read_lobe_xyz: c"), _ptr(out, C.c_double)), "drt_read_lobe_xyz")
        return out

    def read_lobe_bgra(self, c, which=1):
        out = np.empty((self.n_pixels, 4), dtype=np.uint8)
        _check(self.L.drt_read_lobe_bgra(self.ctx, _u32(c, "read_lobe_bgra: c"), int(which), _ptr(out, C.c_uint8)), "drt_read_lobe_bgra")
        return out

    def bind_sensor(self, curves):
        arr, n = _sensor_curves(curves, self.S)
        _check(self.L.drt_bind_sensor(self.ctx, None if arr is None else _ptr(arr, C.c_double), n), "drt_bind_sensor")
        self.n_sensor = n

    def read_sensor_film(self):
        n = getattr(self, "n_sensor", 0)
        px = np.empty((self.n_pixels, n + 1), dtype=np.float64)
        av = np.empty((self.n_pixels, n), dtype=np.float64)
        va = np.empty((self.n_pixels, n), dtype=np.float64)
        _check(self.L.drt_read_sensor_film(self.ctx, _ptr(px, C.c_double), _ptr(av, C.c_double), _ptr(va, C.c_double)), "drt_read_sensor_film")
        return px, av, va

    def sensor_film_device_ptrs(self):
        a, b, c = C.c_void_p(), C.c_void_p(), C.c_void_p()
        _check(self.L.drt_sensor_film_device_ptrs(self.ctx, C.byref(a), C.byref(b), C.byref(c)), "drt_sensor_film_device_ptrs")
        return a.value, b.value, c.value

    def read_sensor_bgra(self, which, matrix):
        n = getattr(self, "n_sensor", 0)
        if n == 0:
            _check(self.L.drt_read_sensor_bgra(self.ctx, int(which), None, None), "drt_read_sensor_bgra")
        m = _sensor_matrix(matrix, n)
        out = np.empty((self.n_pixels, 4), dtype=np.uint8)
        _check(self.L.drt_read_sensor_bgra(self.ctx, int(which), _ptr(m, C.c_double), _ptr(out, C.c_uint8)), "drt_read_sensor_bgra")
        return out

    def read_hit_indices(self, num_samples):
        n = self.n_pixels * num_samples
        out = np.empty((n, int(self.params.max_depth)), dtype=np.int32)
        _check(self.L.drt_read_hit_indices(self.ctx, _ptr(out, C.c_int32), n), "drt_read_hit_indices")
        return out

    def batch_spp(self):
        return int(self.L.drt_batch_spp(self.ctx))

    def shade_instantiation(self):
        return SHADE_INSTANTIATIONS[int(self.L.drt_shade_instantiation(self.ctx))]

    def shade_closed_lds(self):
        return int(self.L.drt_shade_closed_lds(self.ctx)) == 1

    def stats(self):
        st = Stats()
        _check(self.L.drt_get_stats(self.ctx, C.byref(st)), "drt_get_stats")
        return st

    def render_adaptive(self, min_spp, max_spp, step, rel_error, floor=0.0):
        a = make_adaptive(min_spp, max_spp, step, rel_error, floor)
        _check(self.L.drt_render_adaptive(self.ctx, C.byref(a)), "drt_render_adaptive")
        return {"rounds": a.rounds, "pixels_at_max": a.pixels_at_max, "paths": a.paths}

    def render_adaptive_continue(self, max_spp, step, rel_error, floor=0.0, max_rounds=0):
        a = make_adaptive(2, max_spp, step, rel_error, floor)
        left = C.c_uint32()
        _check(self.L.drt_render_adaptive_continue(self.ctx, C.byref(a), max_rounds, C.byref(left)), "drt_render_adaptive_continue")
        return {"rounds": a.rounds, "pixels_at_max": a.pixels_at_max, "paths": a.paths, "still_active": left.value}

    def denoise(self, radius=5, patch=1, k=1.0, alpha=1.0):
        d = make_denoise(radius, patch, k, alpha)
        _check(self.L.drt_denoise_film(self.ctx, C.byref(d)), "drt_denoise_film")
        return {"unusable": d.unusable, "kernel_ms": d.kernel_ms}

    def read_denoised(self):
        mean = np.empty((self.n_pixels, self.S), dtype=np.float64)
        var = np.empty((self.n_pixels, self.S), dtype=np.float64)
        _check(self.L.drt_read_denoised(self.ctx, _ptr(mean, C.c_double), _ptr(var, C.c_double)), "drt_read_denoised")
        return mean, var

    def read_denoised_bgra(self):
        out = np.empty((self.n_pixels, 4), dtype=np.uint8)
        _check(self.L.drt_read_denoised_bgra(self.ctx, _ptr(out, C.c_uint8)), "drt_read_denoised_bgra")
        return out

    def render_features(self, n_samples=0, first_sample=0, flags=0):
        f = make_features(n_samples, first_sample)
        f.flags = flags
        _check(self.L.drt_render_features(self.ctx, C.byref(f)), "drt_render_features")
        return {"empty_pixels": f.empty_pixels, "rays": f.rays, "kernel_ms": f.kernel_ms}

    def read_features(self):
        mean = np.empty((self.n_pixels, FEATURE_CHANNELS), dtype=np.float64)
        m2 = np.empty((self.n_pixels, FEATURE_CHANNELS), dtype=np.float64)
        ids = np.empty(self.n_pixels, dtype=np.int32)
        _check(self.L.drt_read_features(self.ctx, _ptr(mean, C.c_double), _ptr(m2, C.c_double), _ptr(ids, C.c_int32)), "drt_read_features")
        return mean, m2, ids

    def read_feature_bgra(self, which, lo, hi):
        out = np.empty((self.n_pixels, 4), dtype=np.uint8)
        _check(self.L.drt_read_feature_bgra(self.ctx, int(which), float(lo), float(hi), _ptr(out, C.c_uint8)), "drt_read_feature_bgra")
        return out

    def render_mattes(self, n_samples=0, first_sample=0, flags=0):
        m = make_mattes(n_samples, first_sample)
        m.flags = flags
        _check(self.L.drt_render_mattes(self.ctx, C.byref(m)), "drt_render_mattes")
        return _mattes_report(m)

    def read_mattes(self):
        ids = np.empty((self.n_pixels, MATTE_LAYERS, MATTE_SLOTS), dtype=np.int32)
        counts = np.empty((self.n_pixels, MATTE_LAYERS, MATTE_SLOTS), dtype=np.uint32)
        tail = np.empty((self.n_pixels, 4), dtype=np.uint32)
        _check(self.L.drt_read_mattes(self.ctx, _ptr(ids, C.c_int32), _ptr(counts, C.c_uint32), _ptr(tail, C.c_uint32)), "drt_read_mattes")
        return ids, counts, tail

    def read_matte(self, layer, id_list):
        lst = np.ascontiguousarray(id_list, dtype=np.int32).reshape(-1)
        out = np.empty(self.n_pixels, dtype=np.float64)
        _check(self.L.drt_read_matte(self.ctx, int(layer), _ptr(lst, C.c_int32), len(lst), _ptr(out, C.c_double)), "drt_read_matte")
        return out

    def read_matte_bgra(self, layer):
        out = np.empty((self.n_pixels, 4), dtype=np.uint8)
        _check(self.L.drt_read_matte_bgra(self.ctx, int(layer), _ptr(out, C.c_uint8)), "drt_read_matte_bgra")
        return out

    def cast_rays(self, origins, dirs):
        if _is_tensor(origins) or _is_tensor(dirs):
            torch = sys.modules["torch"]
            dev = int(self.params.device)
            o, d = _rays_tensor(origins, "origins", dev), _rays_tensor(dirs, "dirs", dev)
            if o.shape != d.shape:
                raise ValueError("origins and dirs: the same shape")
            hits = torch.empty((o.shape[0], 104), dtype=torch.uint8, device=o.device)
            _check(self.L.drt_cast_rays(self.ctx, o.data_ptr(), d.data_ptr(), o.shape[0], hits.data_ptr(), RAYS_DEVICE), "drt_cast_rays")
# ... 526 lines not shown
```

include/drt_hip.h:

```cpp
#ifndef DRT_HIP_H
#define DRT_HIP_H

#include <stdint.h>

#ifdef __cplusplus
extern "C" {
#endif

#define DRT_MAX_BDSFS 16

enum
{
    DRT_GEO_NONE   = 0,
    DRT_GEO_POINT  = 1,
    DRT_GEO_SPHERE = 2,
    DRT_GEO_PLANE  = 3
};

enum
{
    DRT_FILM_SAMPLE_CENTER = 1,
    DRT_FILM_SAMPLE_RANDOM = 2
};

// ... 77 lines not shown

enum
{
    DRT_MODE_SPECTRAL = 0,
    DRT_MODE_XYZ      = 1
};

typedef struct drt_params
{
    uint32_t width, height;
    uint32_t x0, y0, tile_w, tile_h, row_stride;
    uint32_t spp;
    uint32_t first_sample;
    uint32_t max_depth;
    uint32_t pixel_scheme;
    uint64_t seed;
    uint32_t mode;
    int32_t  device;
    uint32_t batch_spp;
    uint32_t flags;
} drt_params;

#define DRT_BATCH_RESIDENT 0xFFFFFFFFu

enum
{
    DRT_FLAG_RECORD_HITS = 1u,
    DRT_FLAG_FILM_ZERO   = 2u
};

typedef struct drt_stats
{
    uint64_t paths;
    uint64_t closest_hit_scans;
    uint64_t shaded_vertices;
    uint64_t shadow_scans;
    uint64_t rng_draws;
    double   trace_ms;
    double   shade_ms;
    double   total_ms;
    uint64_t record_pool_blocks;
    uint64_t record_pool_peak;
    uint32_t record_block_bytes;
    uint32_t redone_launches;
    uint32_t launches;
    uint32_t path_flags;
    double   min_sample_ms, max_sample_ms, avg_sample_ms;
} drt_stats;

enum
{
    DRT_PATH_BVH        = 1u,
    DRT_PATH_TRACE_TAIL = 2u,
    DRT_PATH_RAYS       = 4u,
    DRT_PATH_RAY_STASH  = 8u
};

typedef struct drt_context drt_context;

const char *drt_last_error(void);
int drt_device_count(void);

drt_context *drt_create(const drt_scene *scene, const drt_camera *camera, const drt_params *params);
void         drt_destroy(drt_context *ctx);
int drt_bind_film(drt_context *ctx, void *d_pixels, void *d_avgs, void *d_vars);
int drt_set_stream(drt_context *ctx, void *hip_stream);
int drt_render(drt_context *ctx, uint32_t first_sample, uint32_t num_samples);
int drt_synchronize(drt_context *ctx);
int drt_reset_film(drt_context *ctx);
int drt_film_device_ptrs(drt_context *ctx, void **d_pixels, void **d_avgs, void **d_vars);
int drt_read_film(drt_context *ctx, double *pixels, double *avgs, double *vars);
int drt_write_film(drt_context *ctx, const double *pixels, const double *avgs, const double *vars);
int drt_read_xyz(drt_context *ctx, double *xyz);
int drt_read_bgra(drt_context *ctx, int which, uint8_t *bgra);
int drt_read_hit_indices(drt_context *ctx, int32_t *dst, uint64_t capacity_paths);
int drt_get_stats(drt_context *ctx, drt_stats *out);
uint32_t drt_batch_spp(drt_context *ctx);

#define DRT_SHADE_GENERAL 0
#define DRT_SHADE_SIMPLE 1
#define DRT_SHADE_CLOSED 2
int drt_shade_instantiation(const drt_context *ctx);
int drt_shade_closed_lds(const drt_context *ctx);

int drt_render_tile(const drt_scene *scene, const drt_camera *camera, const drt_params *params,
                    double *dst_pixels, double *dst_avgs, double *dst_vars, drt_stats *stats);

typedef struct drt_group drt_group;
drt_group *drt_group_create(const drt_scene *scene, const drt_camera *camera, const drt_params *params,
                            const int32_t *devices, uint32_t n_devices);
void     drt_group_destroy(drt_group *g);
uint32_t drt_group_size(drt_group *g);
int drt_group_render(drt_group *g, uint32_t first_sample, uint32_t num_samples);
int drt_group_synchronize(drt_group *g);
int drt_group_read_film(drt_group *g, double *pixels, double *avgs, double *vars);
int drt_group_write_film(drt_group *g, const double *pixels, const double *avgs, const double *vars);
int drt_group_read_bgra(drt_group *g, int which, uint8_t *bgra);
int drt_group_get_stats(drt_group *g, drt_stats *out);
int drt_render_tile_multi(const drt_scene *scene, const drt_camera *camera, const drt_params *params,
                          const int32_t *devices, uint32_t n_devices,
                          double *dst_pixels, double *dst_avgs, double *dst_vars, drt_stats *stats);

typedef struct drt_adaptive
{
    uint32_t min_spp, max_spp, step, flags;
    double   rel_error, floor;
    uint32_t rounds, pixels_at_max;
    uint64_t paths;
} drt_adaptive;
int drt_render_adaptive(drt_context *ctx, drt_adaptive *a);
int drt_read_sample_counts(drt_context *ctx, uint32_t *counts);
int drt_read_active_list(drt_context *ctx, uint32_t *list, uint32_t capacity, uint32_t *count);
int drt_group_render_adaptive(drt_group *g, drt_adaptive *a);
int drt_group_read_sample_counts(drt_group *g, uint32_t *counts);

int drt_render_adaptive_continue(drt_context *ctx, drt_adaptive *a, uint32_t max_rounds, uint32_t *still_active);
int drt_group_render_adaptive_continue(drt_group *g, drt_adaptive *a, uint32_t max_rounds, uint32_t *still_active);

#define DRT_MAP_DEVICE 1u
#define DRT_MAP_ADD    2u
typedef struct drt_sample_map
{
    const uint32_t *targets;
    uint32_t flags;
    uint32_t rounds, pixels_rendered, pixels_above, max_count;
    uint64_t paths;
} drt_sample_map;
int drt_render_sample_map(drt_context *ctx, drt_sample_map *map);
int drt_group_render_sample_map(drt_group *g, drt_sample_map *map);

typedef struct drt_denoise
{
    uint32_t radius, patch, flags;
    uint32_t unusable;
    double   k, alpha;
    double   kernel_ms;
} drt_denoise;
int drt_denoise_film(drt_context *ctx, drt_denoise *d);
int drt_read_denoised(drt_context *ctx, double *mean, double *var);
int drt_read_denoised_bgra(drt_context *ctx, uint8_t *bgra);
int drt_denoise_buffers(const drt_scene *scene, const drt_params *params, drt_denoise *d, const double *pixels, const double *avgs,
                        const double *vars, double *mean, double *var);
int drt_group_denoise(drt_group *g, drt_denoise *d, double *mean, double *var);

#define DRT_FEATURE_CHANNELS 8
typedef struct drt_features
{
    uint32_t n_samples;
    uint32_t first_sample;
    uint32_t flags;
    uint32_t empty_pixels;
    uint64_t rays;
    double   kernel_ms;
} drt_features;
int drt_render_features(drt_context *ctx, drt_features *f);
int drt_read_features(drt_context *ctx, double *mean, double *m2, int32_t *ids);
int drt_read_feature_bgra(drt_context *ctx, int which, double lo, double hi, uint8_t *bgra);
int drt_group_render_features(drt_group *g, drt_features *f, double *mean, double *m2, int32_t *ids);

#define DRT_MATTE_SLOTS   6
#define DRT_MATTE_ID_MISS (-1)
enum { DRT_MATTE_SURFACE = 0, DRT_MATTE_MATERIAL = 1, DRT_MATTE_LAYERS = 2 };
typedef struct drt_mattes
{
    uint32_t n_samples;
    uint32_t first_sample;
// ... 148 lines not shown
```

Before: 2568.

## Add a 512-lane closed-form shade kernel sized for six waves per SIMD

Adds a variant of the closed shade kernel with headers in LDS that launches 512-lane workgroups with launch bounds asking for six waves per SIMD. The LDS plan is recomputed for that shape, and an occupancy query decides whether to select it. To cut register pressure in this variant, the tail pass re-reads ph2 and vignette from LDS instead of keeping them in registers, recomputes the emission term, loads dir_pdf later, and uses scalarised film addressing. The goal is higher occupancy to hide memory latency, at the cost of extra LDS and recomputation work and a new launch path with its own grid cap.

```diff
diff --git a/daily-ray-trace_amd/csrc/drt_kernels.h b/daily-ray-trace_amd/csrc/drt_kernels.h
--- a/daily-ray-trace_amd/csrc/drt_kernels.h
+++ b/daily-ray-trace_amd/csrc/drt_kernels.h
@@ -1936,11 +1936,14 @@
 
 #define XYZ_FILM_WORDS 8
 
+template <bool LEAN>
+struct ShadeTail
+{
 template <bool SPDS_IN_LDS, bool XYZ, bool SIMPLE, bool LIST = false>
 __device__ __forceinline__ void shade_tail_group(const DevScene &sc, const ShadeParams &sp, const double *lds, uint64_t *wave_lds, const uint64_t *__restrict__ records,
                                                  const uint64_t *__restrict__ headers, double *__restrict__ film_pixels,
                                                  double *__restrict__ film_avgs, double *__restrict__ film_vars, uint64_t chunk_base,
-                                                 uint64_t chunk_end, uint32_t lane, const bool closed, const bool closed_lds = false)
+                                                 uint64_t chunk_end, uint32_t lane, const bool closed, const bool closed_lds = false) const
 {
     const uint32_t S = sc.S;
     const uint32_t vw = sp.vertex_words;
@@ -1962,7 +1965,10 @@
     uint64_t slot = 0;
     const uint64_t *vcur = records;
     const bool one_light = sp.n_lights == 1u;
-    const double em0 = spd_at(table, S, one_light ? sp.light0_em_spd : 0u, lam);
+    const double em0_held = LEAN ? 0.0 : spd_at(table, S, one_light ? sp.light0_em_spd : 0u, lam);
+    uint32_t e_cur = 0;
+#define TAIL_EM0 (LEAN ? spd_at(table, S, one_light ? sp.light0_em_spd : 0u, made_again<LEAN>(lam)) : em0_held)
+#define TAIL_PH2 (LEAN ? wave_lds[e_cur * 3u + 2u] : ph2)
     auto deep_blocks = [&](uint32_t vertex) -> uint64_t { return vertex >= 2u * REC_BLOCK_VERTICES ? headers[slot * REC_HEADER_WORDS + 3] : 0ull; };
     for (uint32_t s0 = sp.tail_staged ? sp.n_samples : 0u; s0 < sp.n_samples; s0 += win)
     {
@@ -2024,8 +2030,12 @@
                     const uint32_t ge = e / n_win, off = e - ge * n_win;
                     slot = (chunk_base + ge) * (uint64_t)sp.batch + s0 + off;
                     ph0 = w[0];
+                    if constexpr (LEAN) e_cur = e;
+                    else
+                    {
                     vignette = word_as_double(w[1]);
                     ph2 = w[2];
+                    }
                     n_shaded = (uint32_t)(ph0 & 0xFFFFu);
                     const uint32_t k = ((uint32_t)(ph0 >> 16) >> HDR_TERM_RESUME_SHIFT) & HDR_TERM_RESUME_MASK;
                     v = k;
@@ -2036,9 +2046,9 @@
                         const double *at = sp.tail_stage + (slot * R + j);
                         dst = at[0];
                         throughput = at[shade_const().sp.tail_resume - sp.tail_stage];
-                        vcur = path_vertex(records, sp.block_words, vw, ph2, deep_blocks(k), k);
+                        vcur = path_vertex(records, sp.block_words, vw, LEAN ? w[2] : ph2, deep_blocks(k), k);
                     }
-                    else vcur = records + (uint64_t)(uint32_t)ph2 * sp.block_words;
+                    else vcur = records + (uint64_t)(uint32_t)(LEAN ? w[2] : ph2) * sp.block_words;
                     busy = true;
                 }
                 next_task += (uint32_t)__popcll(want);
@@ -2068,7 +2078,7 @@
                             double reflectance = diffuse_pi * a_in + 0.0;
                             reflectance = (glossy * spec) * a_in + reflectance;
                             contribution = contribution + reflectance;
-                            contribution = contribution * em0;
+                            contribution = contribution * TAIL_EM0;
                             contribution = contribution * c;
                         }
                     }
@@ -2080,7 +2090,7 @@
                         double reflectance = diffuse_pi * a_in + 0.0;
                         reflectance = (glossy * spec) * a_in + reflectance;
                         double lit = 0.0 + reflectance;
-                        lit = lit * em0;
+                        lit = lit * TAIL_EM0;
                         lit = lit * c;
                         contribution = ((uint32_t)(lw0 >> 16) & FLAG_VISIBLE) ? lit : 0.0;
                     }
@@ -2103,7 +2113,7 @@
                     reflectance = reflectance * dir_pdf;
                     throughput = throughput * reflectance;
                     v += 1;
-                    if (v < n_shaded) vcur = (v & (REC_BLOCK_VERTICES - 1u)) != 0u ? vcur + vw : path_vertex(records, sp.block_words, vw, ph2, deep_blocks(v), v);
+                    if (v < n_shaded) vcur = (v & (REC_BLOCK_VERTICES - 1u)) != 0u ? vcur + vw : path_vertex(records, sp.block_words, vw, TAIL_PH2, deep_blocks(v), v);
                 }
             }
             else if (n_general > 0)
@@ -2112,7 +2122,7 @@
                 {
                     const uint64_t *vrec = vcur;
                     const uint64_t list = vrec[0], w1 = vrec[1], w2 = vrec[2];
-                    const double on_dot = word_as_double(vrec[3]), dir_pdf = word_as_double(vrec[4]);
+                    const double on_dot = word_as_double(vrec[3]), dir_pdf = LEAN ? 0.0 : word_as_double(vrec[4]);
                     const uint32_t num_bdsfs = (uint32_t)(w1 & 0xFFu);
                     const uint32_t sflags = (uint32_t)(w1 >> 8) & 0xFFu;
                     const uint32_t i_diffuse = (uint32_t)(w1 >> 16) & 0xFFFFu, i_glossy = (uint32_t)(w1 >> 32) & 0xFFFFu;
@@ -2136,8 +2146,11 @@
                             contribution = contribution * word_as_double(lrec[1]);
                         }
                         dst = dst + throughput * contribution;
+                        double dir_pdf_late = 0.0;
+                        if constexpr (LEAN) dir_pdf_late = word_as_double(vrec[4]);
                         double reflectance = eval(sflags, vrec + 5);
-                        reflectance = reflectance * dir_pdf;
+                        if constexpr (LEAN) reflectance = reflectance * dir_pdf_late;
+                        else reflectance = reflectance * dir_pdf;
                         throughput = throughput * reflectance;
                     };
                     const bool glass = !SIMPLE && num_bdsfs == 2u && list == DRT_LIST_GLASS;
@@ -2168,22 +2181,28 @@
                                                               word_as_double(a[2]), word_as_double(a[3]), flags, paired);
                         });
                     v += 1;
-                    if (v < n_shaded) vcur = (v & (REC_BLOCK_VERTICES - 1u)) != 0u ? vcur + vw : path_vertex(records, sp.block_words, vw, ph2, deep_blocks(v), v);
+                    if (v < n_shaded) vcur = (v & (REC_BLOCK_VERTICES - 1u)) != 0u ? vcur + vw : path_vertex(records, sp.block_words, vw, TAIL_PH2, deep_blocks(v), v);
                 }
             }
             if (busy && v >= n_shaded)
             {
                 if (((uint32_t)(ph0 >> 16) & HDR_TERM_MASK) == 1u) dst = dst + throughput * spd_at(table, S, (uint32_t)(ph0 >> 32) & 0xFFFFu, lam);
-                sp.tail_stage[slot * R + j] = dst * vignette;
+                sp.tail_stage[slot * R + j] = dst * (LEAN ? word_as_double(wave_lds[e_cur * 3u + 1u]) : vignette);
                 busy = false;
             }
         }
         __builtin_amdgcn_wave_barrier();
     }
     uint32_t j_b = j;
+    uint32_t g_b = g;
+    if constexpr (LEAN)
+    {
+        const uint32_t lane_b = made_again<true>(lane);
+        g_b = lane_b / R;
+        j_b = lane_b - g_b * R;
+    }
     asm volatile("" : "+v"(j_b));
     const uint32_t lam_b = sp.tail_first + j_b;
-    uint32_t g_b = g;
     asm volatile("" : "+v"(g_b));
     const uint64_t pix_b = chunk_base + g_b;
     const uint64_t pix_f = LIST ? (act ? (uint64_t)sp.pixel_list[pix_b] : 0u) : pix_b;
@@ -2237,10 +2256,13 @@
         pa[lam_b] = f_avg;
         pv[lam_b] = f_var;
     }
-}
-
-
-template <int NSETS, bool SPDS_IN_LDS, bool XYZ, bool DARK, bool SIMPLE, bool LIST, bool CLOSED, bool CLOSED_LDS = false>
+#undef TAIL_EM0
+#undef TAIL_PH2
+}
+};
+
+
+template <int NSETS, bool SPDS_IN_LDS, bool XYZ, bool DARK, bool SIMPLE, bool LIST, bool CLOSED, bool CLOSED_LDS = false, uint32_t BLOCK = SHADE_BLOCK>
 __device__ __forceinline__ void shade_pixels(const DevScene &sc, const ShadeParams &sp, const uint64_t *__restrict__ records,
                                              const uint64_t *__restrict__ headers, double *__restrict__ film_pixels,
                                              double *__restrict__ film_avgs, double *__restrict__ film_vars,
@@ -2253,12 +2275,13 @@
     if (SPDS_IN_LDS)
     {
         const uint32_t spd_words = sc.n_spd * S;
-        for (uint32_t k = threadIdx.x; k < spd_words; k += SHADE_BLOCK) lds[k] = sc.spds[k];
+        for (uint32_t k = threadIdx.x; k < spd_words; k += BLOCK) lds[k] = sc.spds[k];
         __syncthreads();
     }
     const uint32_t lane_k = threadIdx.x & 63u;
     static_assert(!CLOSED_LDS || CLOSED, "the form with headers in LDS is a closed form");
     constexpr bool LDS_HDR = CLOSED_LDS;
+    constexpr bool FILM_SCALAR = LDS_HDR && BLOCK != SHADE_BLOCK;
     uint64_t *rec_lds = (uint64_t *)(lds + (SPDS_IN_LDS ? (size_t)sc.n_spd * S : 0)) + (size_t)(threadIdx.x >> 6) * SHADE_WAVE_LDS_WORDS_FOR(LDS_HDR);
     const uint32_t vw = sp.vertex_words;
     const uint32_t vpr = vw <= 64 ? 64u / vw : 0u;
@@ -2339,6 +2362,14 @@
         {
             const uint32_t lam = 64u * k + lane;
             const bool active = lam < S_main;
+            if constexpr (FILM_SCALAR)
+            {
+                const uint32_t at = made_again<true>(lane) * 8u;
+                f_sum[k] = active ? *(const double *)((const char *)px + at) : 0.0;
+                f_avg[k] = active ? *(const double *)((const char *)pa + at) : 0.0;
+                f_var[k] = active ? *(const double *)((const char *)pv + at) : 0.0;
+                continue;
+            }
             f_sum[k] = (active && !XYZ) ? px[lam] : 0.0;
             f_avg[k] = (active && !XYZ) ? pa[lam] : 0.0;
             f_var[k] = (active && !XYZ) ? pv[lam] : 0.0;
@@ -2904,6 +2935,17 @@
             for (int k = 0; k < NSETS; k += 1)
             {
                 const uint32_t lam = 64u * k + lane;
+                if constexpr (FILM_SCALAR)
+                {
+                    const uint32_t at = made_again<true>(lane) * 8u;
+                    if (lam < S_main)
+                    {
+                        *(double *)((char *)px + at) = f_sum[k];
+                        *(double *)((char *)pa + at) = f_avg[k];
+                        *(double *)((char *)pv + at) = f_var[k];
+                    }
+                    continue;
+                }
                 if (lam < S_main)
                 {
                     px[lam] = f_sum[k];
@@ -2919,7 +2961,7 @@
         {
             __builtin_amdgcn_wave_barrier();
         }
-        if (tail_item && sp.mode != 1u) shade_tail_group<SPDS_IN_LDS, XYZ, SIMPLE, LIST>(sc, sp, (const double *)lds, rec_lds, records, headers, film_pixels, film_avgs, film_vars, chunk_base, chunk_end, made_again<LDS_HDR>(lane), CLOSED, LDS_HDR);
+        if (tail_item && sp.mode != 1u) ShadeTail<FILM_SCALAR>{}.template shade_tail_group<SPDS_IN_LDS, XYZ, SIMPLE, LIST>(sc, sp, (const double *)lds, rec_lds, records, headers, film_pixels, film_avgs, film_vars, chunk_base, chunk_end, made_again<LDS_HDR>(lane), CLOSED, LDS_HDR);
     }
 }
 
@@ -2955,6 +2997,20 @@
                                                                  unsigned long long *__restrict__ work_counter)
 {
     shade_pixels<1, true, false, DARK, false, false, true, true>(sc, sp, records, headers, film_pixels, film_avgs, film_vars, work_counter);
+}
+
+#define SHADE_BLOCK_CLOSED_LDS6 512
+#define SHADE_WAVES_CLOSED_LDS6 (SHADE_BLOCK_CLOSED_LDS6 / 64)
+#ifndef DRT_SHADE_WAVES_CLOSED_LDS6
+#define DRT_SHADE_WAVES_CLOSED_LDS6 6
+#endif
+template <bool DARK>
+__global__ __launch_bounds__(SHADE_BLOCK_CLOSED_LDS6, DRT_SHADE_WAVES_CLOSED_LDS6) void drt_shade_kernel_closed_lds6(DevScene sc, ShadeParams sp, const uint64_t *__restrict__ records,
+                                                                 const uint64_t *__restrict__ headers, double *__restrict__ film_pixels,
+                                                                 double *__restrict__ film_avgs, double *__restrict__ film_vars,
+                                                                 unsigned long long *__restrict__ work_counter)
+{
+    shade_pixels<1, true, false, DARK, false, false, true, true, SHADE_BLOCK_CLOSED_LDS6>(sc, sp, records, headers, film_pixels, film_avgs, film_vars, work_counter);
 }
 #endif
 
diff --git a/daily-ray-trace_amd/csrc/drt_launcher.hip b/daily-ray-trace_amd/csrc/drt_launcher.hip
--- a/daily-ray-trace_amd/csrc/drt_launcher.hip
+++ b/daily-ray-trace_amd/csrc/drt_launcher.hip
@@ -138,6 +138,9 @@
     size_t shade_lds_closed = 0;
     bool   closed_lds = false;
     bool trace_stash = false;
+    size_t shade_lds_closed6 = 0;
+    bool   closed_lds6 = false;
+    int    shade_grid_cap6 = 0;
     int    trace_grid_cap = 0, shade_grid_cap = 0;
     uint32_t trace_chunk_override = 0;
     ShadeOverrides shade_overrides;
@@ -822,6 +825,9 @@
 }
 
 static bool shade_closed_lds(const drt_context *ctx) { return DRT_SHADE_CLOSED_LDS_HEADERS != 0 && ctx->closed_lds && shade_closed(ctx); }
+static bool shade_closed_lds6(const drt_context *ctx) { return ctx->closed_lds6 && shade_closed_lds(ctx); }
+static uint32_t shade_launch_waves(const drt_context *ctx, bool list) { return !list && shade_closed_lds6(ctx) ? SHADE_WAVES_CLOSED_LDS6 : SHADE_WAVES; }
+static uint32_t shade_launch_grid_cap(const drt_context *ctx, bool list) { return (uint32_t)(!list && shade_closed_lds6(ctx) ? ctx->shade_grid_cap6 : ctx->shade_grid_cap); }
 
 template <int NSETS, bool XYZ, bool LIST>
 static int launch_shade_mode(drt_context *ctx, uint32_t grid, const ShadeParams &sp, double *const film[3])
@@ -832,6 +838,16 @@
     hipLaunchKernelGGL((KERNEL<DARK>), dim3(grid), dim3(SHADE_BLOCK), LDS_BYTES, ctx->stream, ctx->dsc, sp, ctx->d_records, \
                        ctx->d_headers, film[0], film[1], film[2], ctx->d_counters + DRT_NUM_COUNTERS + 1)
 #if DRT_SHADE_CLOSED_LDS_HEADERS
+        if (shade_closed_lds6(ctx))
+        {
+#define DRT_LAUNCH_CLOSED6(DARK)                                                                                                                   \
+    hipLaunchKernelGGL((drt_shade_kernel_closed_lds6<DARK>), dim3(grid), dim3(SHADE_BLOCK_CLOSED_LDS6), ctx->shade_lds_closed6, ctx->stream, ctx->dsc, sp, \
+                       ctx->d_records, ctx->d_headers, film[0], film[1], film[2], ctx->d_counters + DRT_NUM_COUNTERS + 1)
+            if (shade_dark(ctx, sp)) DRT_LAUNCH_CLOSED6(true);
+            else DRT_LAUNCH_CLOSED6(false);
+#undef DRT_LAUNCH_CLOSED6
+            return 0;
+        }
         if (shade_closed_lds(ctx))
         {
             if (shade_dark(ctx, sp)) DRT_LAUNCH_CLOSED(drt_shade_kernel_closed_lds, true, ctx->shade_lds_closed);
@@ -1319,6 +1335,12 @@
     ctx->shade_lds = lds_general.group_bytes;
     ctx->shade_lds_closed = lds_closed.group_bytes;
     ctx->closed_lds = lds_closed.groups >= DRT_SHADE_WAVES_CLOSED_LDS * SHADE_SIMDS_PER_CU / SHADE_WAVES && getenv("DRT_NO_CLOSED_LDS") == nullptr;
+    static_assert(SHADE_WAVES_CLOSED_LDS6 == SHADE_LDS_SIX_BLOCK_WAVES && DRT_SHADE_WAVES_CLOSED_LDS6 == SHADE_LDS_SIX_WAVES_PER_SIMD, "the rule's shape is the kernel's");
+    const ShadeLdsPlan lds_closed6 = shade_lds_plan_six(ctx->dsc.n_spd, S, ctx->spds_in_lds, SHADE_WAVE_LDS_WORDS_FOR(true));
+    ctx->shade_lds_closed6 = lds_closed6.group_bytes;
+    const uint32_t groups6 = SHADE_LDS_SIX_GROUPS;
+    int closed_waves_asked = DRT_SHADE_WAVES_CLOSED_LDS6;
+    if (const char *e = getenv("DRT_CLOSED_WAVES")) closed_waves_asked = atoi(e);
     int s_per_cu = 0;
     shade_sets(S, &ctx->shade_sets, &ctx->tail_first, &ctx->tail_count);
     switch (ctx->shade_sets)
@@ -1332,6 +1354,16 @@
     const int s_query = s_per_cu;
     if (shade_closed_lds(ctx)) s_per_cu = std::min(s_per_cu, (int)lds_closed.groups);
     if (s_per_cu < 1) s_per_cu = 1;
+    int s6_query = -1;
+#if DRT_SHADE_CLOSED_LDS_HEADERS
+    if (shade_closed_lds(ctx) && closed_waves_asked >= DRT_SHADE_WAVES_CLOSED_LDS6 && shade_lds_six_fits(lds_closed6))
+    {
+        HIP_TRY(hipOccupancyMaxActiveBlocksPerMultiprocessor(&s6_query, drt_shade_kernel_closed_lds6<true>, SHADE_BLOCK_CLOSED_LDS6, ctx->shade_lds_closed6));
+        ctx->closed_lds6 = s6_query == (int)groups6;
+    }
+#endif
+    ctx->shade_grid_cap6 = prop.multiProcessorCount * (int)groups6;
+    if (const char *e = getenv("DRT_SHADE_BLOCKS_PER_CU")) ctx->shade_grid_cap6 = prop.multiProcessorCount * std::min((int)groups6, std::max(1, atoi(e)));
     if (const char *e = getenv("DRT_SHADE_BLOCKS_PER_CU")) s_per_cu = std::max(1, atoi(e));
     ctx->shade_grid_cap = prop.multiProcessorCount * s_per_cu;
     if (const char *e = getenv("DRT_RESERVE_BLOCKS"))
@@ -1339,6 +1371,7 @@
         int n = std::max(0, atoi(e));
         ctx->trace_grid_cap = std::max(1, ctx->trace_grid_cap - n);
         ctx->shade_grid_cap = std::max(1, ctx->shade_grid_cap - n);
+        ctx->shade_grid_cap6 = std::max(1, ctx->shade_grid_cap6 - n);
     }
     if (const char *e = getenv("DRT_TRACE_CHUNK")) ctx->trace_chunk_override = (uint32_t)std::min(1 << 20, std::max(64, atoi(e) / 64 * 64));
     if (const char *e = getenv("DRT_TAIL_PERIOD")) ctx->shade_overrides.tail_period = (uint32_t)std::max(0, atoi(e));
@@ -1439,6 +1472,11 @@
     if (ctx->tail_count) HIP_TRY(ctx->d_tail_stage.need((size_t)npx * batch * ctx->tail_count));
     if (ctx->tail_count && ctx->tail_resume) HIP_TRY(ctx->d_tail_resume.need((size_t)npx * batch * ctx->tail_count));
     if (const char *e = getenv("DRT_DARK_SKIP")) ctx->dark_skip = ctx->dark_skip_win = atoi(e) != 0;
+    if (getenv("DRT_VERBOSE"))
+        fprintf(stderr, "drt: shade kernel %s; six waves: %s, occupancy query %d workgroups of %d lanes per CU, lds %zu (LDS rule: %u), grid cap %d\n",
+                shade_closed_lds6(ctx) ? "drt_shade_kernel_closed_lds6" : shade_closed_lds(ctx) ? "drt_shade_kernel_closed_lds" : shade_closed(ctx) ? "drt_shade_kernel_closed" : "drt_shade_kernel",
+                shade_closed_lds6(ctx) ? "chosen" : s6_query >= 0 ? "refused by the query" : "not asked", s6_query, SHADE_BLOCK_CLOSED_LDS6, ctx->shade_lds_closed6,
+                lds_closed6.groups, ctx->shade_grid_cap6);
     if (getenv("DRT_VERBOSE"))
         fprintf(stderr, "drt: %d CUs, trace %d blocks/CU (lds %zu), shade %d blocks/CU (%s, occupancy query %d, lds %zu; LDS rule: general %u, closed %u of %zu bytes), batch %u, %.3f blocks/path measured (worst %u), pool %.2f GB\n",
                 prop.multiProcessorCount, per_cu, ctx->trace_lds, s_per_cu, shade_closed_lds(ctx) ? "closed, headers in LDS" : shade_closed(ctx) ? "closed" : "general", s_query,
@@ -1738,7 +1776,8 @@
     sp.sample_base = span.list ? ctx->d_counts : nullptr;
     sp.mode = ctx->debug_shade_mode;
     sp.cmf_rw = ctx->cmf_rw; sp.cmf_x = ctx->cmf_x; sp.cmf_y = ctx->cmf_y; sp.cmf_z = ctx->cmf_z;
-    const ShadeQueue q = shade_queue(g.n_pix, span.n_samples, ctx->tail_count, sp.tail_staged, (uint32_t)ctx->shade_grid_cap, SHADE_WAVES, SHADE_PIXEL_CHUNK,
+    const ShadeQueue q = shade_queue(g.n_pix, span.n_samples, ctx->tail_count, sp.tail_staged, shade_launch_grid_cap(ctx, span.list != nullptr),
+                                     shade_launch_waves(ctx, span.list != nullptr), SHADE_PIXEL_CHUNK,
                                      ctx->shade_overrides);
     if (q.too_large) return fail(-1, "tile too large for the shade work queue");
     sp.chunk = q.chunk;
@@ -2143,6 +2182,13 @@
 {
     if (!ctx) return -1;
     return shade_closed_lds(ctx) ? 1 : 0;
+}
+
+extern "C" int drt_shade_closed_waves(const drt_context *ctx)
+{
+    if (!ctx) return -1;
+    if (!shade_closed(ctx)) return 0;
+    return shade_closed_lds6(ctx) ? DRT_SHADE_WAVES_CLOSED_LDS6 : shade_closed_lds(ctx) ? DRT_SHADE_WAVES_CLOSED_LDS : DRT_SHADE_WAVES_CLOSED;
 }
 
 static int adaptive_check(drt_context *ctx, const drt_adaptive *a, bool held = false)
diff --git a/daily-ray-trace_amd/csrc/drt_shade_lds_rule.h b/daily-ray-trace_amd/csrc/drt_shade_lds_rule.h
--- a/daily-ray-trace_amd/csrc/drt_shade_lds_rule.h
+++ b/daily-ray-trace_amd/csrc/drt_shade_lds_rule.h
@@ -34,4 +34,15 @@
     return p;
 }
 
+#define SHADE_LDS_SIX_BLOCK_WAVES 8u
+#define SHADE_LDS_SIX_WAVES_PER_SIMD 6u
+#define SHADE_LDS_SIX_GROUPS (SHADE_LDS_SIX_WAVES_PER_SIMD * SHADE_SIMDS_PER_CU / SHADE_LDS_SIX_BLOCK_WAVES)
+
+static inline ShadeLdsPlan shade_lds_plan_six(uint32_t n_spd, uint32_t S, bool spds_in_lds, uint32_t wave_words)
+{
+    return shade_lds_plan(n_spd, S, spds_in_lds, SHADE_LDS_SIX_BLOCK_WAVES, wave_words, SHADE_LDS_SIX_WAVES_PER_SIMD);
+}
+
+static inline bool shade_lds_six_fits(const ShadeLdsPlan &p) { return p.groups >= SHADE_LDS_SIX_GROUPS; }
+
 #endif
diff --git a/daily-ray-trace_amd/pydrt.py b/daily-ray-trace_amd/pydrt.py
--- a/daily-ray-trace_amd/pydrt.py
+++ b/daily-ray-trace_amd/pydrt.py
@@ -669,6 +669,9 @@
         if hasattr(L, "drt_shade_closed_lds"):
             L.drt_shade_closed_lds.argtypes = [C.c_void_p]
             L.drt_shade_closed_lds.restype = C.c_int
+        if hasattr(L, "drt_shade_closed_waves"):
+            L.drt_shade_closed_waves.argtypes = [C.c_void_p]
+            L.drt_shade_closed_waves.restype = C.c_int
         if hasattr(L, "drt_update_surfaces"):
             L.drt_set_camera.argtypes = [C.c_void_p, C.POINTER(Camera)]
             L.drt_update_surfaces.argtypes = [C.c_void_p, C.c_void_p, C.c_uint32, C.c_uint32, C.c_uint32]
@@ -756,7 +759,7 @@
 
 SHADE_INSTANTIATIONS = ("general", "simple", "closed")
 
-HIP_SYMBOLS = ["drt_shade_instantiation", "drt_shade_closed_lds",
+HIP_SYMBOLS = ["drt_shade_instantiation", "drt_shade_closed_lds", "drt_shade_closed_waves",
                "drt_last_error", "drt_device_count", "drt_create", "drt_destroy", "drt_bind_film", "drt_set_stream",
                "drt_render", "drt_synchronize", "drt_reset_film", "drt_film_device_ptrs", "drt_read_film", "drt_write_film",
                "drt_read_xyz", "drt_read_bgra", "drt_read_hit_indices", "drt_get_stats", "drt_batch_spp", "drt_render_tile", "drt_selftest_arith",
@@ -1169,6 +1172,9 @@
     def shade_closed_lds(self):
         return int(self.L.drt_shade_closed_lds(self.ctx)) == 1
 
+    def shade_closed_waves(self):
+        return int(self.L.drt_shade_closed_waves(self.ctx))
+
     def stats(self):
         st = Stats()
         _check(self.L.drt_get_stats(self.ctx, C.byref(st)), "drt_get_stats")
diff --git a/include/drt_hip.h b/include/drt_hip.h
--- a/include/drt_hip.h
+++ b/include/drt_hip.h
@@ -183,6 +183,7 @@
 #define DRT_SHADE_CLOSED 2
 int drt_shade_instantiation(const drt_context *ctx);
 int drt_shade_closed_lds(const drt_context *ctx);
+int drt_shade_closed_waves(const drt_context *ctx);
 
 int drt_render_tile(const drt_scene *scene, const drt_camera *camera, const drt_params *params,
                     double *dst_pixels, double *dst_avgs, double *dst_vars, drt_stats *stats);
```

Measured after the change: 2642 (median of 6 runs). 1.03x the previous value.
